# arogozhnikov/demuxalot

Hardware: AMD Instinct MI355X
Metric: EM iterations/sec + barcodes demuxed/sec, 200k bc x 100k SNP x 64 gt (higher is better)
Workload: dtype f32 terms, f64 sums (guarded mode: coarse pass reads the table as f16 and sums in f32; exact redo where the contract is not proven)

## Files before the change

### demuxalot_amd/_lib.py

```python
import ctypes
import os
from ctypes import POINTER, c_char_p, c_double, c_float, c_int, c_int32, c_int64, c_void_p

import numpy as np

_HERE = os.path.dirname(os.path.abspath(__file__))
LIB_PATH = os.environ.get('DEMUXALOT_AMD_LIB') or os.path.join(_HERE, 'libdemux_hip.so')

DMX_F32, DMX_F64 = 0, 1
T_PSTEP, T_ESTEP, T_MSTEP, T_MCOMBINE, T_ALLREDUCE, T_COUNT = 0, 1, 2, 3, 4, 5
TIMER_NAMES = ('pstep', 'estep', 'mstep', 'mcombine', 'allreduce')
HOST_COLLECTIVE = ctypes.CFUNCTYPE(ctypes.c_int, ctypes.c_void_p, ctypes.c_int, ctypes.c_void_p, ctypes.c_int64, ctypes.c_int)
COLL_ALL_REDUCE, COLL_REDUCE_SCATTER, COLL_ALL_GATHER = 0, 1, 2
UNIQUE_ID_BYTES = 128

_P = c_void_p
SIGNATURES = {
    'dmx_last_error': (c_char_p, []),
    'dmx_version': (c_char_p, []),
    'dmx_device_count': (c_int, [POINTER(c_int)]),
    'dmx_create': (c_int, [c_int, POINTER(_P)]),
    'dmx_destroy': (c_int, [_P]),
    'dmx_synchronize': (c_int, [_P]),
    'dmx_pack_calls_host': (c_int, [c_int64, _P, _P, _P, c_int64, _P, _P, _P, _P, _P, _P,
                                    POINTER(c_int64), POINTER(c_int64), _P, _P, _P, _P, _P]),
    'dmx_hash_host': (c_int, [_P, c_int64, c_int32, POINTER(ctypes.c_uint64)]),
    'dmx_set_problem': (c_int, [_P, c_int64, c_int64, c_int32, c_int64, _P, _P, _P, _P]),
    'dmx_pack_and_set_problem': (c_int, [_P, c_int64, c_int64, c_int32, _P, _P, _P, _P, c_int64, _P, _P, _P, _P, _P,
                                         POINTER(c_int64), POINTER(c_int64), _P]),
    'dmx_pack_containers_and_set_problem': (c_int, [_P, c_int64, c_int64, c_int32, _P, _P, _P, _P, _P, c_int32,
                                                    POINTER(c_int64), POINTER(c_int64), _P]),
    'dmx_stage_containers': (c_int, [_P, _P, c_int32]),
    'dmx_pack_staged_and_set_problem': (c_int, [_P, c_int64, c_int64, c_int32, _P, _P, _P, _P, _P, c_int32,
                                                POINTER(c_int64), POINTER(c_int64), _P]),
    'dmx_get_packed_calls': (c_int, [_P, _P, _P, _P, _P]),
    'dmx_set_betas': (c_int, [_P, _P]),
    'dmx_set_prior_betas': (c_int, [_P, _P, c_double, c_int, _P, _P]),
    'dmx_set_addition': (c_int, [_P, _P]),
    'dmx_probs_from_betas': (c_int, [_P, c_float, c_float, _P]),
    'dmx_probs_from_betas_f64': (c_int, [_P, _P, c_float, c_float, _P]),
    'dmx_set_probs': (c_int, [_P, _P]),
    'dmx_estep': (c_int, [_P, c_int, _P, _P, c_int, _P, _P]),
    'dmx_mstep': (c_int, [_P, c_float, _P]),
    'dmx_em': (c_int, [_P, c_int, c_float, c_float, c_int, _P, _P, c_int, c_float, _P, _P, _P]),
    'dmx_run_iterations': (c_int, [_P, c_int, c_float, c_float, c_float]),
    'dmx_get_logits': (c_int, [_P, _P]),
    'dmx_get_probs': (c_int, [_P, _P]),
    'dmx_get_addition': (c_int, [_P, _P]),
    'dmx_get_block': (c_int, [_P, c_int, c_int64, c_int64, c_int64, c_int64, _P]),
    'dmx_get_assignments': (c_int, [_P, _P, _P]),
    'dmx_get_assignments_above': (c_int, [_P, c_float, _P, _P, POINTER(c_int64)]),
    'dmx_get_top_options': (c_int, [_P, c_int32, _P, _P]),
    'dmx_get_option_sums': (c_int, [_P, _P]),
    'dmx_set_keep_molecule_calls': (c_int, [_P, c_int]),
    'dmx_set_molecule_calls': (c_int, [_P, c_int64, _P, _P, _P]),
    'dmx_get_max_pair_count': (c_int, [_P, POINTER(c_int64)]),
    'dmx_estep_snp': (c_int, [_P, c_int, _P, c_int64, _P, c_int, _P, _P]),
    'dmx_mstep_f64': (c_int, [_P, c_double, _P]),
    'dmx_mstep_f64_sums': (c_int, [_P, c_double, _P]),
    'dmx_get_prior_betas': (c_int, [_P, _P]),
    'dmx_get_learnt_betas': (c_int, [_P, _P]),
    'dmx_exchange_slices': (c_int, [c_int64, _P, c_int32, _P, POINTER(c_int64), POINTER(c_int32)]),
    'dmx_comm_unique_id': (c_int, [_P]),
    'dmx_comm_init': (c_int, [_P, c_int, c_int, _P, c_int]),
    'dmx_comm_init_host': (c_int, [_P, c_int, c_int, _P, _P, c_int]),
    'dmx_get_timings': (c_int, [_P, POINTER(c_double), POINTER(c_int64)]),
    'dmx_reset_timings': (c_int, [_P]),
    'dmx_set_phase_timers': (c_int, [_P, c_int]),
    'dmx_set_logits_needed': (c_int, [_P, c_int]),
    'dmx_set_lean_memory': (c_int, [_P, c_int]),
    'dmx_device_bytes': (c_int, [_P, POINTER(c_int64)]),
    'dmx_trim_cache': (c_int, [_P, POINTER(c_int64)]),
    'dmx_release_problem': (c_int, [_P]),
    'dmx_trim_device_caches': (c_int, [c_int, POINTER(c_int64)]),
    'dmx_set_exact_additions': (c_int, [_P, c_int]),
    'dmx_set_estep_mode': (c_int, [_P, c_int]),
    'dmx_set_msteps_expected': (c_int, [_P, c_int64]),
    'dmx_snp_count': (c_int, [_P, _P, c_int32, _P, c_int64, c_int32, c_float, c_int32, POINTER(c_int64)]),
    'dmx_snp_score': (c_int, [_P, c_double, _P, _P, _P, _P, _P, _P]),
    'dmx_snp_select': (c_int, [_P, c_int64, c_int64, _P, POINTER(c_int64)]),
    'dmx_count_reads': (c_int, [_P, _P, _P, c_int64, _P, POINTER(c_int64), POINTER(c_int64)]),
    'dmx_count_reads_fetch': (c_int, [_P, _P, _P]),
    'dmx_coverage_count': (c_int, [_P, _P, c_int32, c_int32, c_int32, _P]),
    'dmx_coverage_candidates': (c_int, [_P, c_double, c_double, c_double, c_double, c_int64, POINTER(c_int64)]),
    'dmx_coverage_fetch_candidates': (c_int, [_P, _P, _P]),
}
DEBUG_SIGNATURES = {
    'dmx_comm_init_emulated': (c_int, [_P, c_int, c_int, c_double, c_double, c_int]),
    'dmx_get_exchange_compact': (c_int, [_P, POINTER(c_int64), POINTER(c_int64), POINTER(c_int64)]),
    'dmx_get_exchange_compact_table': (c_int, [_P, POINTER(c_int64), POINTER(c_int64), POINTER(c_int64)]),
    'dmx_get_guard_probes': (c_int, [_P, POINTER(c_int64), POINTER(c_int64)]),
    'dmx_debug_set_pass_ms': (c_int, [_P, c_double, c_double, c_double]),
    'dmx_get_redo_count': (c_int, [_P, POINTER(c_int64)]),
    'dmx_set_guard_adaptive': (c_int, [_P, c_int]),
    'dmx_set_coarse_pass': (c_int, [_P, c_int]),
    'dmx_set_mstep_incremental': (c_int, [_P, c_int]),
    'dmx_get_mstep_incremental': (c_int, [_P, POINTER(c_int64), POINTER(c_int64), POINTER(c_int64)]),
    'dmx_get_guard_levels': (c_int, [_P, POINTER(c_int32), POINTER(c_int64), POINTER(c_int64), POINTER(c_int64), POINTER(c_double), POINTER(c_double), POINTER(c_double)]),
    'dmx_get_guard_direct': (c_int, [_P, POINTER(c_int32), POINTER(c_int64), POINTER(c_int64), POINTER(c_double), POINTER(c_double)]),
    'dmx_set_estep_schedule': (c_int, [_P, c_int]),
    'dmx_set_estep_dictionary': (c_int, [_P, c_int]),
    'dmx_get_estep_form': (c_int, [_P, POINTER(c_int32), POINTER(c_int32)]),
    'dmx_set_estep_packing': (c_int, [_P, c_int]),
    'dmx_set_mstep_wide_addresses': (c_int, [_P, c_int]),
    'dmx_set_mstep_tiles': (c_int, [_P, c_int]),
    'dmx_get_mstep_form': (c_int, [_P, POINTER(c_int32)]),
    'dmx_get_mstep_tiles_info': (c_int, [_P, POINTER(c_int32), POINTER(c_double)]),
    'dmx_test_logf': (c_int, [_P, _P, _P, c_int64]),
    'dmx_test_logf_hot': (c_int, [_P, _P, _P, c_int64]),
    'dmx_test_expf': (c_int, [_P, _P, _P, c_int64]),
    'dmx_test_log2_hw': (c_int, [_P, _P, _P, c_int64]),
    'dmx_test_softmax': (c_int, [_P, _P, _P, c_int64, c_int64]),
    'dmx_runtime_info': (c_int, [c_char_p, c_int64]),
    'dmx_get_exchange_mode': (c_int, [_P, POINTER(c_int32)]),
    'dmx_get_guard_stats': (c_int, [_P, POINTER(c_int64), POINTER(c_int64), POINTER(c_int64)]),
    'dmx_get_count_reads_timings': (c_int, [_P, POINTER(c_double)]),
    'dmx_count_reads_begin': (c_int, [_P, _P, c_int64, _P]),
    'dmx_count_reads_push': (c_int, [_P, _P, c_int, POINTER(c_int64), POINTER(c_int64)]),
    'dmx_count_reads_end': (c_int, [_P]),
    'dmx_get_count_reads_carry': (c_int, [_P, POINTER(c_int64)]),
    'dmx_get_count_reads_peak_bytes': (c_int, [_P, POINTER(c_int64)]),
    'dmx_set_coverage_form': (c_int, [_P, c_int]),
    'dmx_get_coverage_timings': (c_int, [_P, POINTER(c_double)]),
    'dmx_reads_upload': (c_int, [_P, _P, POINTER(c_int64)]),
    'dmx_reads_release': (c_int, [_P, c_int64]),
    'dmx_reads_info': (c_int, [_P, c_int64, POINTER(c_int64)]),
    'dmx_count_reads_resident': (c_int, [_P, c_int64, _P, c_int64, _P, POINTER(c_int64), POINTER(c_int64)]),
    'dmx_coverage_count_resident': (c_int, [_P, c_int64, c_int32, c_int32, c_int32, _P]),
    'dmx_count_reads_push_resident': (c_int, [_P, c_int64, c_int64, c_int64, c_int, POINTER(c_int64), POINTER(c_int64)]),
    'dmx_get_reads_upload_bytes': (c_int, [_P, POINTER(c_int64)]),
    'dmx_calls_upload': (c_int, [_P, _P, POINTER(c_int64)]),
    'dmx_calls_open': (c_int, [_P, POINTER(c_int64)]),
    'dmx_calls_append_counted': (c_int, [_P, c_int64]),
    'dmx_calls_seal': (c_int, [_P, c_int64]),
    'dmx_calls_concatenate': (c_int, [_P, POINTER(c_int64), c_int32, POINTER(c_int64)]),
    'dmx_calls_view': (c_int, [_P, c_int64, _P]),
    'dmx_calls_info': (c_int, [_P, c_int64, POINTER(c_int64)]),
    'dmx_calls_fetch': (c_int, [_P, c_int64, _P, _P]),
    'dmx_calls_release': (c_int, [_P, c_int64]),
    'dmx_calls_barcode_counts': (c_int, [_P, c_int64, c_int64, _P, _P]),
    'dmx_stage_device_containers': (c_int, [_P, _P, c_int32]),
    'dmx_snp_count_device': (c_int, [_P, _P, c_int32, _P, c_int64, c_int32, c_float, c_int32, POINTER(c_int64)]),
    'dmx_get_calls_transfer_bytes': (c_int, [_P, POINTER(c_int64)]),
    'dmx_get_donor_readout': (c_int, [_P, _P, _P, _P, _P, _P, _P, _P]),
    'dmx_get_allowed_mass': (c_int, [_P, _P, _P, _P, _P]),
    'dmx_estep_pools': (c_int, [_P, c_int, c_int32, _P, _P, _P, _P, _P, _P, _P, _P, _P, _P]),
    'dmx_estep_pools_resident': (c_int, [_P, c_int, c_int32, _P, _P, _P, _P, _P, _P, _P, _P, _P, _P]),
    'dmx_em_pools': (c_int, [_P, c_int, c_float, c_float, c_int, c_int32, _P, _P, _P, _P, _P, c_float, _P, _P, _P, _P, _P, _P]),
}

COVERAGE_STAGES = ('upload', 'walk', 'window', 'accumulate', 'filter', 'top_n')
COVERAGE_ATOMIC, COVERAGE_TILED = 0, 1
CALLS_INFO = ('n_molecules', 'n_snp_calls', 'nbytes', 'sealed')
READS_INFO = ('n_reads', 'n_cigar_ops', 'n_bases', 'nbytes', 'reference_length')
COUNT_READS_STAGES = ('upload', 'walk', 'molecules', 'duplicates', 'observations', 'fold', 'order')


class CallContainerStruct(ctypes.Structure):
    _fields_ = [('snp_calls', _P), ('n_snp_calls', c_int64), ('molecules', _P), ('n_molecules', c_int64), ('chrom', c_int32)]


class DecodedReadsStruct(ctypes.Structure):
    _fields_ = [('n_reads', c_int64), ('reference_start', _P), ('compressed_cb', _P), ('compressed_ub', _P), ('p_misaligned', _P),
                ('alignment_score', _P), ('cigar_begin', _P), ('n_cigar', _P), ('seq_begin', _P), ('l_seq', _P),
                ('n_cigar_ops', c_int64), ('cigar', _P), ('n_bases', c_int64), ('seq', _P), ('qual', _P)]


_lib = None


class DemuxHipError(RuntimeError):
    pass


def load():
    global _lib
    if _lib is None:
        if not os.path.exists(LIB_PATH):
            raise DemuxHipError(
                f'{LIB_PATH} is missing: build it with `python -c "import __graft_entry__ as g; g.build()"` '
                f'or `make -C demuxalot_amd/csrc`. demuxalot_amd has no CPU fallback.')
        os.environ.setdefault('HSA_ENABLE_IPC_MODE_LEGACY', '0')
        lib = ctypes.CDLL(LIB_PATH)
        for name, (res, args) in {**SIGNATURES, **DEBUG_SIGNATURES}.items():
            fn = getattr(lib, name)
            fn.restype = res
            fn.argtypes = args
        _lib = lib
    return _lib

# ... 35 lines not shown
```

### demuxalot_amd/csrc/dmx_api.cpp

```cpp
#include <dlfcn.h>
#include <hip/hip_runtime.h>
#include <rccl/rccl.h>

#include <array>
#include <chrono>
#include <functional>

#include <algorithm>
#include <mutex>
#include <cmath>
#include <cstdio>
#include <cstdlib>
#include <cstring>
#include <string>
#include <vector>

#include "dmx_ctx.h"
#include "dmx_host.h"

using namespace dmx::host;

extern "C" {

static int begin_problem(dmx_ctx *c, int64_t B, int64_t V, int32_t G, const int32_t *v2snp, std::vector<int> &snp_ptr,
// ... 345 lines not shown
        if (ms[i] < 0.0) continue;
        const unsigned ticks = (unsigned)std::min(ms[i] * (double)khz, 1.0e9);
        HIP_TRY(hipMemcpy(c->d_guard_count.p + word[i], &ticks, sizeof(unsigned), hipMemcpyHostToDevice));
        if (i == 2) {
            const unsigned measured = ticks != 0u;
            HIP_TRY(hipMemcpy(c->d_guard_count.p + dmx::GS_E_MEASURED, &measured, sizeof(unsigned), hipMemcpyHostToDevice));
        }
    }
    return 0;
}

int dmx_set_estep_dictionary(dmx_ctx *c, int mode)
{
    if (!c) return fail(DMX_ERR_INVALID, "null context");
    if (mode < 0 || mode > 2) return fail(DMX_ERR_INVALID, "dictionary mode must be 0, 1 or 2");
    c->dict_mode = mode;
    return 0;
}

int dmx_set_estep_packing(dmx_ctx *c, int on)
{
    if (!c) return fail(DMX_ERR_INVALID, "null context");
    if (on < 0 || on > 3) return fail(DMX_ERR_INVALID, "packing mode must be 0 .. 3");
    c->estep_packing = on;
    return 0;
}

int dmx_get_estep_form(dmx_ctx *c, int32_t *form, int32_t *distinct_values)
{
    if (!c) return fail(DMX_ERR_INVALID, "null context");
    if (form) *form = c->estep_form;
    if (distinct_values) *distinct_values = c->dict_distinct;
    return 0;
}

int dmx_set_estep_schedule(dmx_ctx *c, int tiled)
{
    if (!c) return fail(DMX_ERR_INVALID, "null context");
    if (tiled < 0 || tiled > 2) return fail(DMX_ERR_INVALID, "schedule must be 0, 1 or 2");
    c->tiled_estep = tiled;
    return 0;
}

int dmx_get_redo_count(dmx_ctx *c, int64_t *count)
{
    DMX_TRY(bind(c));
    if (!count) return fail(DMX_ERR_INVALID, "null argument");
    unsigned n[2] = {0, 0};
    if (c->d_n_redo.p) {
        HIP_TRY(hipMemcpyAsync(n, c->d_n_redo.p, 2 * sizeof(unsigned), hipMemcpyDeviceToHost, c->stream));
        HIP_TRY(hipStreamSynchronize(c->stream));
    }
    *count = (int64_t)n[0] + (int64_t)n[1];
    return 0;
}

int dmx_set_mstep_tiles(dmx_ctx *c, int enable)
{
    if (!c) return fail(DMX_ERR_INVALID, "null context");
    if (enable < 0 || enable > 2) return fail(DMX_ERR_INVALID, "dmx_set_mstep_tiles: 0 never, 1 when it pays, 2 always");
    c->mstep_tiles = enable;
    return 0;
}

int dmx_set_msteps_expected(dmx_ctx *c, int64_t n)
{
    if (!c) return fail(DMX_ERR_INVALID, "null context");
    c->msteps_expected = n > 0 ? (long long)n : 0;
    return 0;
}

int dmx_get_mstep_tiles_info(dmx_ctx *c, int32_t *built, double *build_ms)
{
    if (!c) return fail(DMX_ERR_INVALID, "null context");
    if (built) *built = c->n_mt > 0 ? 1 : 0;
    if (build_ms) *build_ms = c->n_mt > 0 ? c->mt_build_ms : 0.0;
    return 0;
}

int dmx_get_mstep_form(dmx_ctx *c, int32_t *form)
{
    if (!c || !form) return fail(DMX_ERR_INVALID, "null argument");
    *form = c->mstep_form;
    return 0;
}

int dmx_set_mstep_wide_addresses(dmx_ctx *c, int wide)
{
    if (!c) return fail(DMX_ERR_INVALID, "null context");
    c->mstep_wide = wide != 0;
    return 0;
}

int dmx_set_betas(dmx_ctx *c, const float *prior)
{
    DMX_TRY(bind(c));
    DMX_TRY(need(c, c->have_problem, "dmx_set_problem before dmx_set_betas"));
    if (!prior && c->V > 0) return fail(DMX_ERR_INVALID, "null betas");
    HIP_TRY(hipMemcpyAsync(c->d_prior.p, prior, sizeof(float) * c->V * c->G, hipMemcpyHostToDevice, c->stream));
    HIP_TRY(hipStreamSynchronize(c->stream));
    c->have_betas = true;
    c->have_raw = false;
    return 0;
}

int dmx_set_prior_betas(dmx_ctx *c, const float *raw_betas, double default_prior, int add_data_prior,
                        const int64_t *mol_per_variant, float *prior_out)
{
    DMX_TRY(bind(c));
    DMX_TRY(need(c, c->have_problem, "a resident problem before dmx_set_prior_betas"));
    const long long V = c->V;
    const int G = c->G;
    if (V > 0 && !raw_betas) return fail(DMX_ERR_INVALID, "null betas");
    const size_t vg = (size_t)V * G;
    c->have_raw = false;
    if (!c->d_raw.p) DMX_TRY(dev_alloc(c, c->d_raw, vg));
    float *d_raw = c->d_raw.p, *d_bsum = nullptr;
    HIP_TRY(hipMalloc((void **)&d_bsum, (size_t)(V ? V : 1) * sizeof(float)));
    int rc = 0;
    do {
        if (vg && hipMemcpyAsync(d_raw, raw_betas, vg * sizeof(float), hipMemcpyHostToDevice, c->stream) != hipSuccess) {
            rc = fail(DMX_ERR_HIP, "upload of the raw betas failed");
            break;
        }
        const unsigned long long *n_mol = nullptr;
        if (add_data_prior) {
            if (mol_per_variant) {
                dev_free(c, c->d_mol);
                if ((rc = dev_alloc(c, c->d_mol, (size_t)V)) != 0) break;
                if (V && hipMemcpyAsync(c->d_mol.p, mol_per_variant, sizeof(long long) * V, hipMemcpyHostToDevice, c->stream) != hipSuccess) {
                    rc = fail(DMX_ERR_HIP, "upload of the molecule counts failed");
                    break;
                }
            } else if (!c->d_mol.p) {
                rc = fail(DMX_ERR_INVALID, "add_data_prior needs molecule counts: pass them or install the problem with dmx_pack_and_set_problem");
                break;
            }
            n_mol = c->d_mol.p;
        }
        const hipError_t e = dmx::launch_prior_betas(c->stream, d_raw, d_bsum, n_mol, c->d_v2snp.p, c->d_snp_ptr.p, c->d_snp_vars.p, V, G,
                                    default_prior, c->d_prior.p);
        if (e != hipSuccess) {
            rc = fail(DMX_ERR_HIP, "prior betas kernel: %s", hipGetErrorString(e));
            break;
        }
        if (prior_out && vg && hipMemcpyAsync(prior_out, c->d_prior.p, vg * sizeof(float), hipMemcpyDeviceToHost, c->stream) != hipSuccess) {
            rc = fail(DMX_ERR_HIP, "download of the prior betas failed");
            break;
        }
        if (hipStreamSynchronize(c->stream) != hipSuccess) rc = fail(DMX_ERR_HIP, "synchronisation failed");
    } while (false);
    (void)hipStreamSynchronize(c->stream);
    (void)hipFree(d_bsum);
    if (rc == 0) c->have_betas = c->have_raw = true;
    return rc;
}

int dmx_get_prior_betas(dmx_ctx *c, float *out)
{
    DMX_TRY(bind(c));
    DMX_TRY(need(c, c->have_problem && c->have_betas, "prior betas (dmx_set_betas / dmx_set_prior_betas) before dmx_get_prior_betas"));
    DMX_TRY(copy_out(c, out, c->d_prior.p, (size_t)c->V * c->G));
    HIP_TRY(hipStreamSynchronize(c->stream));
    return 0;
}

// ... 123 lines not shown
```

### demuxalot_amd/csrc/dmx_ctx.h

```cpp
#pragma once
#include <hip/hip_runtime.h>
#include <rccl/rccl.h>

#include <map>
#include <mutex>
#include <string>
#include <unordered_map>
#include <utility>
#include <vector>

#include "dmx_internal.h"
#include "kernels.h"

using dmx::fail;

#define HIP_TRY(expr)                                                                                   \
    do {                                                                                                \
        hipError_t _e = (expr);                                                                         \
        if (_e != hipSuccess) return fail(DMX_ERR_HIP, "%s failed: %s", #expr, hipGetErrorString(_e)); \
    } while (0)

#define DMX_TRY(expr)         \
    do {                      \
        int _s = (expr);      \
// ... 98 lines not shown
    DevBuf<unsigned> d_coarse_stream;
    DevBuf<long long> d_coarse_bin_ptr;
    DevBuf<double> d_log2_keep;
    bool coarse_ready = false;
    bool prob16_valid = false;
    int coarse_pass = 1;
    int lean_memory = 0;
    bool logits_needed = true;
    bool logits_readable = true;
    float p_clip_lo = 0.0f;
    DevBuf<double> d_add64, d_partial;
    DevBuf<float> d_logits, d_post;
    DevBuf<unsigned long long> d_nz;
    DevBuf<unsigned long long> d_redo;
    DevBuf<unsigned> d_n_redo;
    bool mstep_wide = false;
    DevBuf<uint2> d_mt_stream;
    DevBuf<long long> d_mt_ptr;
    DevBuf<int> d_mt_first;
    DevBuf<int> d_mt_order;
    DevBuf<int> d_mt_shift;
    DevBuf<unsigned char> d_mt_shift_v;
    DevBuf<unsigned long long> d_acc64;
    DevBuf<float> d_prev_post;
    DevBuf<uint2> d_prev_first;
    DevBuf<int> d_incr_list;
    DevBuf<unsigned char> d_incr_touched;
    DevBuf<unsigned> d_incr_state;
    int incr_parity = 0;
    bool incr_valid = false;
    float incr_power = 0.0f;
    int mstep_incremental = 1;
    long long mstep_incr_launches = 0;
    long long n_mt = 0;
    std::vector<long long> h_col_ptr;
    int mt_tv = 0;
    bool mt_tried = false;
    bool mt_shift_tried = false;
    int mstep_tiles = 1;
    long long msteps_done = 0;
    long long incr_rows = 0;
    DevBuf<unsigned char> d_incr_map;
    DevBuf<uint2> d_slice_rec;
    DevBuf<long long> d_slice_ptr;
    bool slice_index_tried = false;
    bool incr_heavy = false;
    int msteps_ahead = 0;
    long long msteps_expected = 0;
    double mt_build_ms = 0.0;
    int mstep_form = 0;
    DevBuf<int> d_sum_plan;
    long long sum_plan_k = -1;
    int sum_plan_values = 0;
    int item_calls = 1024;
    bool exact_additions = true;
    int estep_mode = DMX_ESTEP_EXACT;
    DevBuf<unsigned> d_guard_count;
    int guard_adaptive = 1;
    DevBuf<int> d_guard_list;
    DevBuf<int> d_guard_sub;
    unsigned guard_sub_cap = 0;
    long long guard_rows_total = 0;
    bool guard_ran = false;
    int tiled_estep = 1;
    int dict_mode = 1;
    bool add_is_zero = true;
    bool dict_candidate = false;
    int estep_form = 0;
    int estep_packing = 1;
    long long max_row_calls = 0;
    int n_simd = 0;
    long long long_row_calls[3] = {0, 0, 0};
    long long n_long_rows[3] = {0, 0, 0};
    int dict_distinct = 0;
    DevBuf<float> d_dict;
    DevBuf<unsigned char> d_codes;
    DevBuf<unsigned char> d_dtab;
    DevBuf<unsigned> d_dict_stat;
    DevBuf<dmx::EstepSegment> d_segs;
    DevBuf<int> d_split_first;
    DevBuf<double> d_seg_sums;
    long long n_segs = 0, n_split = 0;
    float nz_floor = 0.0f;
    DevBuf<uint2> d_first;
    DevBuf<unsigned long long> d_dense_calls;
    bool dense_stat_valid = false;
    DevBuf<float> d_pen;
    DevBuf<unsigned> d_pairs;
    DevBuf<unsigned> d_pair_blocks;
    int n_pair_blocks = 0;
    DevBuf<unsigned char> d_prior_logits;
    DevBuf<int> d_best;
    DevBuf<float> d_bestp;
    DevBuf<int> d_u_variant, d_u_cb;
    DevBuf<float> d_u_p;
    DevBuf<long long> d_u_count;
    long long n_u = 0;
    DevBuf<unsigned long long> d_mol;
    bool keep_molecule_calls = false;
    DevBuf<int> d_mc_variant;
    DevBuf<float> d_mc_e;
    DevBuf<long long> d_mc_start;
    unsigned mc_max_count = 0;
    DevBuf<double> d_logits64, d_post64;
    bool have_post64 = false;
    DevBuf<unsigned char> d_scratch;
    DevBuf<unsigned long long> d_sd_pos;
    DevBuf<int> d_sd_counts;
    DevBuf<double> d_sd_imp;
    long long sd_P = -1;
    int sd_D = 0;
    bool sd_scored = false;
    DevBuf<unsigned char> d_cr_molecules;
    DevBuf<unsigned char> d_cr_calls;
    long long cr_molecules = -1, cr_calls = 0;
    double cr_stage_ms[dmx::COUNT_READS_STAGES] = {};
    int64_t cr_peak_bytes = 0;
    long long cr_carried = 0;
    DevBuf<int> d_crs_positions;
    DevBuf<double> d_crs_table;
    ReadColumns crs_carry;
    int crs_state = 0;
    long long crs_P = 0;
    long long crs_molecules = 0;
    long long crs_previous_start = 0;
    bool crs_has_previous = false;
    DevBuf<int> d_cov_counts;
    DevBuf<int> d_cov_cand_pos;
    DevBuf<int> d_cov_cand_counts;
    long long cov_W = -1, cov_start = 0, cov_candidates = -1;
    int coverage_form = DMX_COVERAGE_TILED;
    double cov_stage_ms[dmx::COVERAGE_STAGES] = {};
    std::map<int64_t, ResidentReads> resident_reads;
    int64_t reads_upload_bytes = 0;
    std::map<int64_t, ResidentCalls> resident_calls;
    int64_t calls_transfer_bytes[2] = {0, 0};

    ncclComm_t comm = nullptr;
    dmx_host_collective host_coll = nullptr;
    void *host_user = nullptr;
    void *h_stage = nullptr;
    size_t h_stage_bytes = 0;
    bool emulated = false;
    double emu_link_gbps = 50.0, emu_latency_us = 10.0;
    bool in_group = false, group_paid = false;
    double group_ns = 0.0;
    bool emu_table_filled = false;
    double emu_ticks_per_ns = 0.1;
    bool attached() const { return comm != nullptr || host_coll != nullptr || emulated; }
    int rank = 0, nranks = 1, reduce_dtype = DMX_F64;
    bool sliced = false;
    bool add_partial = false;
    long long slice_rows = 0;
    long long prob_rows = 0;
    std::vector<long long> cut;
    std::vector<int> h_v2snp;
    DevBuf<int> d_prow;
    DevBuf<int> d_row_variant;
    bool mshard = false;
    long long rows_pad = 0, rows_total = 0;
    DevBuf<uint2> d_first_g;
    DevBuf<unsigned long long> d_nz_g;
    DevBuf<float> d_post_g;
    bool post_gathered = false;
    bool emu_post_filled = false;
    DevBuf<unsigned> d_post_compact;
// ... 129 lines not shown
```

### demuxalot_amd/csrc/dmx_runtime.cpp

```cpp
#include <dlfcn.h>
#include <hip/hip_runtime.h>
#include <rccl/rccl.h>

#include <array>
#include <chrono>
#include <functional>

#include <algorithm>
#include <mutex>
#include <cmath>
#include <cstdio>
#include <cstdlib>
#include <cstring>
#include <string>
#include <vector>

#include "dmx_ctx.h"
#include "dmx_host.h"

using namespace dmx::host;

namespace dmx {
static thread_local std::string g_last_error;

// ... 677 lines not shown
    c->boundary = nullptr;
    for (int slot = 0; slot < DMX_T_COUNT; slot++) timer_flush(c, slot);
    for (TimerStamp *s : c->idle_stamps) {
        (void)hipEventDestroy(s->ev);
        delete s;
    }
    (void)hipStreamDestroy(c->stream);
    delete c;
    return 0;
}

int dmx_synchronize(dmx_ctx *c)
{
    DMX_TRY(bind(c));
    HIP_TRY(hipStreamSynchronize(c->stream));
    return 0;
}

int dmx_release_problem(dmx_ctx *c)
{
    DMX_TRY(bind(c));
    HIP_TRY(hipStreamSynchronize(c->stream));
    release_problem(c);
    release_snp_detection(c);
    release_count_reads(c);
    release_count_reads_stream(c);
    release_coverage(c);
    dmx::release_staged_calls(c);
    return 0;
}

int dmx_trim_device_caches(int device, int64_t *released_bytes)
{
    int n = 0;
    if (hipGetDeviceCount(&n) != hipSuccess || device < 0 || device >= n) return fail(DMX_ERR_INVALID, "device %d out of range", device);
    HIP_TRY(hipSetDevice(device));
    const size_t freed = trim_device_caches(device);
    if (released_bytes) *released_bytes = (int64_t)freed;
    return 0;
}

int dmx_trim_cache(dmx_ctx *c, int64_t *released_bytes)
{
    DMX_TRY(bind(c));
    size_t before = 0;
    {
        std::lock_guard<std::mutex> own(c->cache_lock);
        before = c->idle_bytes;
    }
    ctx_trim(c, 0);
    before += retired_trim(c->device);
    if (released_bytes) *released_bytes = (int64_t)before;
    return 0;
}

int dmx_set_phase_timers(dmx_ctx *c, int on)
{
    if (!c) return fail(DMX_ERR_INVALID, "null ctx");
    c->phase_timers = on != 0;
    c->boundary = nullptr;
    return 0;
}

int dmx_get_timings(dmx_ctx *c, double *ms, int64_t *launches)
{
    DMX_TRY(bind(c));
    HIP_TRY(hipStreamSynchronize(c->stream));
    for (int s = 0; s < DMX_T_COUNT; s++) {
        timer_flush(c, s);
        if (ms) ms[s] = (c->timers[s].launches > 0 && c->timers[s].timed == 0) ? -1.0 : c->timers[s].ms;
        if (launches) launches[s] = c->timers[s].launches;
    }
    return 0;
}

int dmx_reset_timings(dmx_ctx *c)
{
    DMX_TRY(bind(c));
    HIP_TRY(hipStreamSynchronize(c->stream));
    if (c->d_guard_count.p) HIP_TRY(hipMemsetAsync(c->d_guard_count.p + dmx::GS_PENDING, 0, 4 * sizeof(unsigned), c->stream));
    if (c->d_guard_count.p) HIP_TRY(hipMemsetAsync(c->d_guard_count.p + dmx::GS_COARSE_STEPS, 0, 2 * sizeof(unsigned), c->stream));
    if (c->d_incr_state.p) HIP_TRY(hipMemsetAsync(c->d_incr_state.p + 2 * dmx::IS_WORDS, 0, sizeof(unsigned) * 3, c->stream));
    c->guard_rows_total = 0;
    for (int s = 0; s < DMX_T_COUNT; s++) {
        timer_flush(c, s);
        c->timers[s].ms = 0.0;
        c->timers[s].launches = 0;
        c->timers[s].timed = 0;
    }
    return 0;
}

int dmx_device_bytes(dmx_ctx *c, int64_t *bytes)
{
    if (!c || !bytes) return fail(DMX_ERR_INVALID, "null argument");
    *bytes = c->bytes;
    return 0;
}

}
```

### demuxalot_amd/csrc/dmx_steps.cpp

```cpp
#include <dlfcn.h>
#include <hip/hip_runtime.h>
#include <rccl/rccl.h>

#include <array>
#include <chrono>
#include <functional>

#include <algorithm>
#include <mutex>
#include <cmath>
#include <cstdio>
#include <cstdlib>
#include <cstring>
#include <string>
#include <vector>

#include "dmx_ctx.h"
#include "dmx_host.h"
#include "estep_plan.h"
#include "estep_pools.h"
#include "mstep_plan.h"

using namespace dmx::host;

// ... 213 lines not shown
    c->dict_candidate = !with_addition || c->add_is_zero;
    return 0;
}

namespace ep = dmx::eplan;
static_assert(ep::MODE_EXACT == DMX_ESTEP_EXACT && ep::MODE_FAST == DMX_ESTEP_FAST && ep::MODE_GUARDED == DMX_ESTEP_GUARDED, "estep_plan.h: Mode");

static ep::Facts estep_facts(const dmx_ctx *c, int with_doublets, bool with_prior, bool logits_kept)
{
    ep::Facts f{};
    f.mode = (ep::Mode)c->estep_mode;
    f.with_doublets = with_doublets != 0;
    f.with_prior = with_prior;
    f.logits_kept = logits_kept;
    f.G = c->G;
    f.K = c->K;
    f.B = c->B;
    f.table_rows = c->prob_rows;
    f.schedule = c->tiled_estep;
    f.n_bins = c->n_bins;
    f.tile_stream = c->d_tile_stream.p != nullptr;
    f.coarse_ready = c->coarse_ready;
    f.coarse_pass = c->coarse_pass;
    f.guard_adaptive = c->guard_adaptive != 0;
    f.lean_memory = c->lean_memory != 0;
    f.lo = c->p_clip_lo;
    f.prob16_valid = c->prob16_valid;
    f.sliced = c->sliced;
    f.table_lists = c->prob_list_words != 0;
    f.dict_mode = c->dict_mode;
    f.dict_candidate = c->dict_candidate;
    f.call_rows = c->d_call_rows.p != nullptr;
    f.records_below_4g = ((unsigned long long)c->n_pairs + dmx::CALL_PAD_PAIRS) * sizeof(dmx::CallPair) < (1ull << 32);
    f.packing = c->estep_packing;
    f.row_statistic = c->max_row_calls > 0;
    for (int k = 0; k < 3; k++) f.n_long_rows[k] = c->n_long_rows[k];
    f.segments = c->n_segs > 0;
    f.n_pair_blocks = with_doublets && c->d_pair_blocks.p != nullptr ? c->n_pair_blocks : 0;
    return f;
}

int prepare_dictionary(dmx_ctx *c, bool pairs, dmx::EstepArgs &a, int *form)
{
    const ep::Facts f = estep_facts(c, pairs, false, true);
    *form = DMX_FORM_DIRECT;
    a.dict_n = 0;
    c->dict_distinct = 0;
    if (!ep::dictionary_admissible(f)) return 0;
    const int G = c->G;
    const long long K = c->K, rows = c->prob_rows;
    const size_t code_pitch = (size_t)dmx::dict_code_pitch(G);
    DMX_TRY(dev_grow(c, c->d_dict, (size_t)rows * dmx::DICT_CAP));
    DMX_TRY(dev_grow(c, c->d_codes, (size_t)rows * code_pitch));
    if (!c->d_dict_stat.p) DMX_TRY(dev_alloc(c, c->d_dict_stat, (size_t)1));
    HIP_TRY(dmx::launch_build_dict(c->stream, c->d_prob.p, rows, G, c->d_dict.p, c->d_codes.p, c->d_dict_stat.p));
    unsigned distinct = 0;
    HIP_TRY(hipMemcpyAsync(&distinct, c->d_dict_stat.p, sizeof(unsigned), hipMemcpyDeviceToHost, c->stream));
    HIP_TRY(hipStreamSynchronize(c->stream));
    c->dict_distinct = (int)distinct;
    const size_t pitch = ep::dictionary_candidate_form(f, distinct) == ep::DICT_LANE ? (size_t)dmx::dict_table_pitch((int)distinct, (int)K, f.with_doublets) : 0;
    switch (ep::dictionary_form(f, distinct, pitch)) {
    case ep::DICT_NONE:
        return 0;
    case ep::DICT_BLOCK:
        a.dict_n = (int)distinct;
        a.dict = c->d_dict.p;
        a.codes = c->d_codes.p;
        *form = DMX_FORM_DICT_BLOCK;
        return 0;
    case ep::DICT_LANE:
        break;
    }
    const size_t need_bytes = (size_t)rows * pitch;
    DMX_TRY(dev_grow(c, c->d_dtab, need_bytes));
    HIP_TRY(dmx::launch_pack_rows(c->stream, c->d_dict.p, c->d_codes.p, c->d_pairs.p, rows, G, (int)K, f.with_doublets, (int)distinct, c->d_dtab.p));
    a.dict_n = (int)distinct;
    a.dtab = c->d_dtab.p;
    a.dtab_pitch = (int)pitch;
    a.dtab_bytes = (unsigned)need_bytes;
    *form = DMX_FORM_DICT;
    return 0;
}

static void fill_estep_args(dmx_ctx *c, dmx::EstepArgs &a, int with_doublets, bool with_prior, int prior_dtype, float power)
{
    a.pair_ptr = c->d_pair_ptr.p;
    a.order = c->d_bc_order.p;
    a.pairs = c->d_call_pairs.p;
    a.call_rows = c->d_call_rows.p;
    const unsigned long long rec_bytes = ((unsigned long long)c->n_pairs + dmx::CALL_PAD_PAIRS) * sizeof(dmx::CallPair);
    a.pairs_bytes = rec_bytes < (1ull << 32) ? (unsigned)rec_bytes : 0u;
    a.prob = c->d_prob.p;
    a.prob16 = nullptr;
    a.guard_accum = 0.0f;
    a.guard_alt_per_call = 0.0f;
    a.guard_alt_accum = 0.0f;
    a.guard_main_coarse = 0;
    a.opt_pairs = c->d_pairs.p;
    a.pair_blocks = with_doublets ? c->d_pair_blocks.p : nullptr;
    a.n_pair_blocks = with_doublets ? c->n_pair_blocks : 0;
    a.sum_plan = c->d_sum_plan.p;
    a.sum_plan_values = c->sum_plan_values;
    a.pen = c->d_pen.p;
    a.prior = with_prior ? c->d_prior_logits.p : nullptr;
    a.prior_dtype = prior_dtype;
    a.logits = c->d_logits.p;
    a.post = c->d_post.p;
    const size_t row_base = c->mshard ? (size_t)c->rank * (size_t)c->rows_pad : 0;
    a.nz = c->mshard ? c->d_nz_g.p + row_base * ((c->G + 63) / 64) : c->d_nz.p;
    a.first = c->G <= 64 ? (c->mshard ? c->d_first_g.p + row_base : c->d_first.p) : nullptr;
    a.post_singlets = c->mshard ? c->d_post_g.p + row_base * c->G : nullptr;
    a.dense_calls = c->G <= 64 ? c->d_dense_calls.p : nullptr;
    a.nz_floor = power == 2.0f ? dmx::NZ_FLOOR_SQUARE : 0.0f;
    a.B = c->B;
    a.prob_bytes = (unsigned)((unsigned long long)c->prob_rows * c->G * 4ull);
    a.G = c->G;
    a.K = c->K;
    a.fast = 0;
    a.guard = 0;
    a.guard_per_call = ep::GUARD_PER_CALL_PLAIN;
    a.guard_count = c->d_guard_count.p;
    a.guard_list = c->d_guard_list.p;
    a.guard_sub = c->d_guard_sub.p;
    a.guard_sub_cap = c->guard_sub_cap;
    a.order_count = nullptr;
    a.direct = nullptr;
    a.order_direct = nullptr;
    a.segs = nullptr;
    a.n_segs = c->n_segs;
    a.n_split = c->n_split;
    a.split_first = c->d_split_first.p;
    a.seg_sums = c->d_seg_sums.p;
    a.tiled = c->tiled_estep;
    a.n_bins = 0;
    a.bin_rows_cap = c->bin_rows_cap;
    a.bin_order = c->d_bin_order.p;
    a.bin_rows = c->d_bin_rows.p;
    a.bin_ptr = c->d_bin_ptr.p;
    a.tile_stream = c->d_tile_stream.p;
    a.coarse_stream = nullptr;
    a.coarse_bin_ptr = nullptr;
    a.log2_keep = nullptr;
    a.n_long = 0;
    a.dict_n = 0;
    a.dtab = nullptr;
    a.dtab_bytes = 0;
    a.dtab_pitch = 0;
    a.dict = nullptr;
    a.codes = nullptr;
}

static void set_walk(const dmx_ctx *c, dmx::EstepArgs &a, ep::Walk walk, bool coarse = false)
{
    const ep::Handover h = ep::handover(walk, coarse);
    a.tile_stream = c->d_tile_stream.p;
    if (!h.bins) a.n_bins = 0;
    if (h.coarse_records) {
        a.coarse_stream = c->d_coarse_stream.p;
        a.coarse_bin_ptr = c->d_coarse_bin_ptr.p;
        a.log2_keep = c->d_log2_keep.p;
    }
    if (h.prob16) a.prob16 = c->d_prob16.p;
}

static int guarded_estep(dmx_ctx *c, ep::Facts &f, dmx::EstepArgs &a)
{
    const bool capable = ep::coarse_capable(f, f.lo), allow_coarse = ep::allow_coarse(f), release = ep::lean_release_due(f);
    const float fine_allowance_found = ep::fine_allowance(f, ep::walk(f));
    if (ep::coarse_build_due(f)) {
        const int cpg = ep::coarse_calls_per_gather(f.K), bpr = ep::coarse_batches_per_record(cpg);
        const size_t words = (((size_t)c->n_pairs / 4 + (size_t)c->n_bins * (bpr - 1)) / bpr + 1) * (size_t)(cpg * 16);
        DMX_TRY(dev_alloc(c, c->d_coarse_stream, words));
        DMX_TRY(dev_alloc(c, c->d_coarse_bin_ptr, (size_t)c->n_bins + 1));
        DMX_TRY(dev_alloc(c, c->d_log2_keep, (size_t)c->B));
        HIP_TRY(dmx::launch_build_coarse_stream(c->stream, c->d_tile_stream.p, c->d_bin_ptr.p, c->n_bins, a.prob_bytes, cpg, c->d_coarse_bin_ptr.p, c->d_coarse_stream.p,
                                                c->d_bin_rows.p, c->bin_rows_cap, c->d_log2_keep.p));
        c->coarse_ready = f.coarse_ready = true;
        if (release) {
            dev_free(c, c->d_tile_stream);
            dev_free(c, c->d_call_rows);
            a.tile_stream = nullptr;
            a.call_rows = nullptr;
            f.tile_stream = f.call_rows = false;
        }
    }
    if (allow_coarse) DMX_TRY(ensure_prob16(c));
    HIP_TRY(dmx::launch_guard_begin(c->stream, c->d_guard_count.p, c->B, c->K, c->guard_adaptive, capable, allow_coarse));
    a.guard = 1;
    a.guard_per_call = fine_allowance_found;
    a.order_direct = c->d_bc_order.p;
    a.guard_main_coarse = 0;
    a.guard_alt_per_call = capable ? dmx::GUARD_PER_CALL_COARSE : 0.0f;
    a.guard_alt_accum = capable ? dmx::GUARD_ACCUM_F32 : 0.0f;
    if (allow_coarse) {
        if (ep::prob16_conversion_due(f)) {
            const bool kept = ep::prob16_stays_valid(f);
// ... 68 lines not shown
            HIP_TRY(dmx::launch_estep_packed(c->stream, a));
            form = DMX_FORM_PACKED;
        } else if (ep::guarded(f)) {
            DMX_TRY(guarded_estep(c, f, a));
        } else {
            set_walk(c, a, ep::walk(f));
            HIP_TRY(dmx::launch_estep(c->stream, a, f.with_doublets));
        }
    }
    c->estep_form = form;
    if (a.dense_calls) HIP_TRY(dmx::launch_sum_dense(c->stream, c->d_dense_calls.p, c->guard_ran ? c->d_guard_count.p : nullptr));
    else if (c->guard_ran) HIP_TRY(dmx::launch_guard_stamp(c->stream, c->d_guard_count.p, dmx::GS_T_END));
    timer_end(c, DMX_T_ESTEP, ev);
    c->have_post = true;
    c->logits_readable = logits_kept;
    return 0;
}

static int ensure_incremental_state(dmx_ctx *c, bool sharded, long long incr_rows, float power)
{
    if (!c->d_acc64.p) {
        c->incr_rows = incr_rows;
        DMX_TRY(dev_alloc(c, c->d_acc64, (size_t)c->V * c->G));
        DMX_TRY(dev_alloc(c, c->d_prev_post, (size_t)incr_rows * c->G));
        DMX_TRY(dev_alloc(c, c->d_prev_first, (size_t)incr_rows));
        DMX_TRY(dev_alloc(c, c->d_incr_list, (size_t)incr_rows));
        if (sharded) {
            DMX_TRY(dmx::build_slice_row_index(c));
            if (c->d_slice_rec.p == nullptr) {
                DMX_TRY(dev_alloc(c, c->d_incr_map, (size_t)incr_rows));
                HIP_TRY(hipMemsetAsync(c->d_incr_map.p, 0, (size_t)incr_rows, c->stream));
            }
        }
        DMX_TRY(dev_alloc(c, c->d_incr_touched, (size_t)c->V));
        DMX_TRY(dev_alloc(c, c->d_incr_state, (size_t)(3 * dmx::IS_WORDS)));
        HIP_TRY(hipMemsetAsync(c->d_incr_state.p, 0, sizeof(unsigned) * 3 * dmx::IS_WORDS, c->stream));
        HIP_TRY(hipMemsetAsync(c->d_incr_touched.p, 0, (size_t)c->V, c->stream));
        c->incr_valid = false;
    }
    if (!c->incr_valid || c->incr_power != power) {
        HIP_TRY(hipMemsetAsync(c->d_incr_state.p, 0, sizeof(unsigned) * 2 * dmx::IS_WORDS, c->stream));
        if (c->mstep_incremental == 2 && !c->attached()) {
            const unsigned on[2] = {1u, 1u};
            HIP_TRY(hipMemsetAsync(c->d_acc64.p, 0, sizeof(unsigned long long) * (size_t)c->V * c->G, c->stream));
            HIP_TRY(hipMemsetAsync(c->d_prev_post.p, 0, sizeof(float) * (size_t)incr_rows * c->G, c->stream));
            HIP_TRY(hipMemsetAsync(c->d_prev_first.p, 0xFF, sizeof(uint2) * (size_t)incr_rows, c->stream));
            HIP_TRY(hipMemsetAsync(c->d_add.p, 0, sizeof(float) * (size_t)c->V * c->G, c->stream));
            HIP_TRY(hipMemcpyAsync(c->d_incr_state.p + dmx::IS_VALID, &on[0], sizeof(unsigned), hipMemcpyHostToDevice, c->stream));
            HIP_TRY(hipMemcpyAsync(c->d_incr_state.p + dmx::IS_FORCE, &on[1], sizeof(unsigned), hipMemcpyHostToDevice, c->stream));
            HIP_TRY(hipStreamSynchronize(c->stream));
        }
        c->incr_parity = 0;
        c->incr_valid = true;
        c->incr_power = power;
    }
    return 0;
}

int run_mstep(dmx_ctx *c, float power)
{
    const bool mshard = c->mshard;
    const size_t row_base = mshard ? (size_t)c->rank * (size_t)c->rows_pad : 0;
    const int Wn = (c->G + 63) / 64;
    dmx::MstepArgs a;
    a.order = c->d_item_order.p;
    a.item_start = c->d_item_start.p;
    a.item_len = c->d_item_len.p;
    a.calls = c->d_csc.p;
    a.post = mshard ? c->d_post_g.p : c->d_post.p;
    a.nz = mshard ? c->d_nz_g.p : c->d_nz.p;
    a.first = mshard ? c->d_first_g.p : c->d_first.p;
    const unsigned long long rows = mshard ? (unsigned long long)c->rows_total : (unsigned long long)c->B;
    a.K = mshard ? c->G : c->K;
    a.first_bytes = 8ull * rows;
    a.wide = c->mstep_wide;
    a.post_bytes = rows * (unsigned long long)a.K * 4ull;
    a.partial = c->d_partial.p;
    a.n_items = c->n_items;
    a.G = c->G;
    a.square = (power == 2.0f);
    a.power = power;
    a.dense_calls = c->dense_stat_valid && a.post_bytes < (1ull << 32) ? c->d_dense_calls.p : nullptr;
    a.total_calls = 2ull * (unsigned long long)c->n_pairs;
    if (!a.square && c->nz_floor != 0.0f) {
        HIP_TRY(dmx::launch_rebuild_nz(c->stream, c->d_post.p, c->B, c->K, c->G, 0.0f, (mshard ? c->d_nz_g.p : c->d_nz.p) + row_base * Wn,
                                       c->G <= 64 ? (mshard ? c->d_first_g.p : c->d_first.p) + row_base : nullptr));
        c->nz_floor = 0.0f;
        c->post_gathered = false;
    }
    DMX_TRY(gather_posteriors(c));
    c->add_is_zero = false;
    TimerSpan ev{nullptr, nullptr};
    SpanGuard ev_guard{c, &ev};
    mplan::Facts f{};
    f.mstep_tiles = c->mstep_tiles;
    f.mstep_incremental = c->mstep_incremental;
    f.exact_additions = c->exact_additions;
    f.G = c->G;
    f.has_calls = c->n_csc > 0;
    f.power = power;
    f.attached = c->attached();
    f.mshard = c->mshard;
    f.sliced = c->sliced;
    f.reduce_f64 = c->reduce_dtype == DMX_F64;
    f.has_call_pairs = c->d_call_pairs.p != nullptr;
    f.has_item_variant = c->d_item_variant.p != nullptr;
    f.has_shift_v = c->d_mt_shift_v.p != nullptr;
    f.has_incr_state = c->d_incr_state.p != nullptr;
    f.has_slice_rec = c->d_slice_rec.p != nullptr;
    f.n_mt = c->n_mt;
    f.mt_tried = c->mt_tried;
    f.msteps_done = c->msteps_done;
    f.msteps_ahead = c->msteps_ahead;
    f.msteps_expected = c->msteps_expected;
    f.incr_heavy = c->incr_heavy;
    f.rows_total = c->rows_total;
    if (mplan::probe_due(f)) {
        unsigned full_passes = 0;
        HIP_TRY(hipMemcpyAsync(&full_passes, c->d_incr_state.p + 2 * dmx::IS_WORDS + 3, sizeof(unsigned), hipMemcpyDeviceToHost, c->stream));
        HIP_TRY(hipStreamSynchronize(c->stream));
        f.incr_heavy = c->incr_heavy = mplan::heavy_after_probe(f, full_passes);
    }
    if (c->msteps_expected > 0) c->msteps_expected--;
    c->msteps_done++;
    const mplan::Range own = mplan::variant_range(f, c->cut.data(), c->rank, c->V);
    if (mplan::build_due(f)) {
        HIP_TRY(hipStreamSynchronize(c->stream));
        const auto t0 = std::chrono::steady_clock::now();
        DMX_TRY(dmx::build_mstep_tiles(c, own.v0, own.v1));
        c->mt_build_ms = std::chrono::duration<double, std::milli>(std::chrono::steady_clock::now() - t0).count();
        f.n_mt = c->n_mt;
    }
    if (mplan::shifts_wanted(f)) DMX_TRY(dmx::plan_mstep_shifts(c));
    f.has_shift_v = c->d_mt_shift_v.p != nullptr;
    const mplan::Launch plan = mplan::launch(f);
    const mplan::Dest dest = mplan::destination(f);
    const bool incremental = plan.incr != mplan::INCR_NONE, sharded = plan.incr == mplan::INCR_SHARDED;
    const long long incr_rows = sharded ? c->rows_total : c->B;
    if (incremental) DMX_TRY(ensure_incremental_state(c, sharded, incr_rows, power));
    else c->incr_valid = false;
    f.has_slice_rec = c->d_slice_rec.p != nullptr;
    const bool by_rows = sharded && mplan::sharded_by_row_index(f);
    a.item_variant = c->d_item_variant.p;
    a.item_ptr = c->d_item_ptr.p;
    a.prow = dest.exchange_buffer ? c->d_prow.p : nullptr;
    a.out32 = dest.f64 ? nullptr : dest.exchange_buffer ? (float *)c->d_exch.p : c->d_add.p;
    a.out64 = !dest.f64 ? nullptr : dest.exchange_buffer ? (double *)c->d_exch.p : c->d_add64.p;
    a.redo_cap = c->d_redo.n;
    a.tiles_done = plan.form == 2;
    a.incr_total = !sharded ? 0ull : by_rows ? (unsigned long long)c->n_csc : 2ull * (unsigned long long)incr_rows;
    dmx::MTileArgs tiles{};
    if (a.tiles_done) {
        tiles.stream = c->d_mt_stream.p;
        tiles.ptr = c->d_mt_ptr.p;
        tiles.first = c->d_mt_first.p;
        tiles.order = c->d_mt_order.p;
        tiles.shift = c->d_mt_shift.p;
        tiles.n_tiles = c->n_mt;
        tiles.tv = c->mt_tv;
    }
    dmx::MIncrArgs incr{};
    if (incremental) {
        incr.state = c->d_incr_state.p + c->incr_parity * dmx::IS_WORDS;
        incr.next = c->d_incr_state.p + (c->incr_parity ^ 1) * dmx::IS_WORDS;
        c->incr_parity ^= 1;
        incr.counters = c->d_incr_state.p + 2 * dmx::IS_WORDS;
        incr.acc64 = c->d_acc64.p;
        incr.prev = c->d_prev_post.p;
        incr.prev_first = c->d_prev_first.p;
        incr.list = c->d_incr_list.p;
        incr.touched = c->d_incr_touched.p;
        incr.shift_v = c->d_mt_shift_v.p;
        incr.pairs = sharded ? nullptr : c->d_call_pairs.p;
        incr.call_rows = sharded ? nullptr : c->d_call_rows.p;
        incr.pair_ptr = sharded ? nullptr : c->d_pair_ptr.p;
        incr.changed_map = sharded ? c->d_incr_map.p : nullptr;
        incr.rec = sharded ? c->d_slice_rec.p : nullptr;
        incr.rec_ptr = by_rows ? c->d_slice_ptr.p : nullptr;
        incr.row_variant = plan.row_variant ? c->d_row_variant.p : nullptr;
        incr.B = incr_rows;
        incr.V = c->V;
        incr.floor = dmx::mincr_floor(power);
        tiles.acc64 = c->d_acc64.p;
        tiles.incr_state = incr.state;
        c->mstep_incr_launches++;
    }
    const bool fixed = plan.incr == mplan::INCR_WORK_ITEMS;
    a.fixed_shift_v = fixed ? c->d_mt_shift_v.p : nullptr;
    a.fixed_acc64 = fixed ? c->d_acc64.p : nullptr;
    a.fixed_state = fixed ? incr.state : nullptr;
    timer_begin(c, DMX_T_MSTEP, &ev);
    HIP_TRY(incremental ? dmx::launch_mstep_incremental(c->stream, a, a.tiles_done ? &tiles : nullptr, incr)
            : a.tiles_done ? dmx::launch_mstep_tiles(c->stream, a, tiles) : dmx::launch_mstep(c->stream, a));
    c->mstep_form = plan.form;
    timer_end(c, DMX_T_MSTEP, ev);
    timer_begin(c, DMX_T_MCOMBINE, &ev);
    HIP_TRY(dmx::launch_mcombine(c->stream, a, c->d_item_ptr.p, own.v0, own.v1, a.prow, a.out32, a.out64, c->exact_additions ? c->d_redo.p : nullptr,
                                 c->d_n_redo.p, nullptr, true));
    timer_end(c, DMX_T_MCOMBINE, ev);
    int rc = 0;
    if (dest.then != mplan::EXCH_NONE) timer_begin(c, DMX_T_ALLREDUCE, &ev);
    if (dest.then == mplan::EXCH_REDUCE_SCATTER) {
        rc = coll_reduce_scatter(c, c->d_exch.p, c->d_recv.p, (size_t)c->slice_rows * c->G, dest.f64, c->stream);
        if (rc == 0)
            HIP_TRY(dmx::launch_store_slice(c->stream, c->d_recv.p, dest.f64, c->cut[c->rank], c->cut[c->rank + 1] - c->cut[c->rank], c->G, c->d_add.p));
    } else if (dest.then == mplan::EXCH_ALL_REDUCE) {
        rc = coll_all_reduce(c, dest.f64 ? (void *)c->d_add64.p : (void *)c->d_add.p, (size_t)c->V * c->G, dest.f64);
        if (rc == 0 && dest.f64) HIP_TRY(dmx::launch_f64_to_f32(c->stream, c->d_add64.p, c->d_add.p, (long long)c->V * c->G));
    }
    if (dest.then != mplan::EXCH_NONE) timer_end(c, DMX_T_ALLREDUCE, ev);
    if (rc == 0 && dest.slice_only) c->add_partial = c->nranks > 1;
    return rc;
}

}
}

extern "C" {

// ... 136 lines not shown
        if (p < -1 || p >= n_pools) return fail(DMX_ERR_INVALID, "%s: pool_of_barcode[%lld] = %d is outside [-1, %d)", who, b, p, (int)n_pools);
        const long long options = p < 0 ? 0 : plan.opt_ptr[(size_t)p + 1] - plan.opt_ptr[(size_t)p];
        if (row_ptr[b + 1] - row_ptr[b] != options)
            return fail(DMX_ERR_INVALID, "%s: row_ptr gives barcode %lld %lld entries, its pool has %lld options", who, b,
                        (long long)(row_ptr[b + 1] - row_ptr[b]), options);
    }
    plan.pair_penalty = pair_penalty;
    plan.pool_of_barcode = pool_of_barcode;
    plan.row_ptr = row_ptr;
    plan.logits_out = logits_out;
    plan.probs_out = probs_out;
    plan.best_option = best_option;
    plan.best_prob = best_prob;
    plan.doublet_mass = doublet_mass;
    return 0;
}

static int begin_dense_pools(dmx_ctx *c)
{
    const std::vector<float> zeros((size_t)std::max(c->G, 1), 0.0f);
    DMX_TRY(ensure_options(c, 0, zeros.data()));
    const size_t bg = (size_t)c->B * c->G;
    HIP_TRY(hipMemsetAsync(c->d_post.p, 0, sizeof(float) * (bg ? bg : 1), c->stream));
    c->have_post = false;
    return 0;
}

int dmx_estep_pools(dmx_ctx *c, int with_doublets, int32_t n_pools, const int64_t *pool_start, const int32_t *pool_donors,
                    const float *pair_penalty, const int32_t *pool_of_barcode, const int64_t *row_ptr, float *logits_out,
                    float *probs_out, int32_t *best_option, float *best_prob, double *doublet_mass)
{
    DMX_TRY(bind(c));
    dmx::PoolsPlan plan;
    DMX_TRY(plan_pools(c, "dmx_estep_pools", false, false, with_doublets, n_pools, pool_start, pool_donors, pair_penalty, pool_of_barcode, row_ptr,
                       logits_out, probs_out, best_option, best_prob, doublet_mass, plan));
    return dmx::run_estep_pools(c, plan);
}

int dmx_estep_pools_resident(dmx_ctx *c, int with_doublets, int32_t n_pools, const int64_t *pool_start, const int32_t *pool_donors,
                             const float *pair_penalty, const int32_t *pool_of_barcode, const int64_t *row_ptr, float *logits_out,
                             float *probs_out, int32_t *best_option, float *best_prob, double *doublet_mass)
{
    DMX_TRY(bind(c));
    dmx::PoolsPlan plan;
    DMX_TRY(plan_pools(c, "dmx_estep_pools_resident", true, false, with_doublets, n_pools, pool_start, pool_donors, pair_penalty, pool_of_barcode,
                       row_ptr, logits_out, probs_out, best_option, best_prob, doublet_mass, plan));
    DMX_TRY(begin_dense_pools(c));
    dmx::PoolsRunPtr run;
    DMX_TRY(dmx::prepare_estep_pools(c, plan, true, run));
    DMX_TRY(dmx::launch_estep_pools_pass(c, *run, 2.0f));
    return dmx::read_back_estep_pools(c, *run);
}

int dmx_mstep(dmx_ctx *c, float power, float *addition_out)
{
    DMX_TRY(bind(c));
    DMX_TRY(need(c, c->have_problem && c->have_post, "dmx_estep before dmx_mstep"));
    DMX_TRY(run_mstep(c, power));
    if (addition_out) DMX_TRY(ensure_full_addition(c));
    DMX_TRY(copy_out(c, addition_out, c->d_add.p, (size_t)c->V * c->G));
    HIP_TRY(hipStreamSynchronize(c->stream));
    return 0;
}

int dmx_em(dmx_ctx *c, int n_iterations, float lo, float hi, int with_doublets, const float *penalties,
           const void *prior_logits, int prior_dtype, float power, float *logits_out, float *probs_out,
           float *addition_out)
{
    DMX_TRY(bind(c));
    DMX_TRY(need(c, c->have_problem && c->have_betas, "dmx_set_problem + dmx_set_betas before dmx_em"));
    if (n_iterations < 1) return fail(DMX_ERR_INVALID, "n_iterations must be >= 1");
    if (!penalties) return fail(DMX_ERR_INVALID, "null penalties");
    DMX_TRY(ensure_options(c, with_doublets, penalties));
    DMX_TRY(upload_prior_logits(c, prior_logits, prior_dtype));
    const size_t vg = (size_t)c->V * c->G;
    HIP_TRY(hipMemsetAsync(c->d_add.p, 0, sizeof(float) * (vg ? vg : 1), c->stream));
    c->incr_valid = false;
    c->add_is_zero = true;
    c->add_partial = false;
    const bool keep_last = c->logits_needed || logits_out != nullptr;
    for (int it = 0; it < n_iterations; it++) {
        const bool kept = it + 1 == n_iterations && keep_last;
        DMX_TRY(run_pstep(c, lo, hi, true, !kept && it > 0 && ep::coarse_capable(estep_facts(c, with_doublets, false, kept), lo)));
        DMX_TRY(run_estep(c, with_doublets, it == 0 && prior_logits != nullptr, prior_dtype, power, kept));
        if (it + 1 < n_iterations) {
            c->msteps_ahead = n_iterations - 1 - it;
            const int rc_m = run_mstep(c, power);
            c->msteps_ahead = 0;
            if (rc_m) return rc_m;
        }
    }
    const size_t bk = (size_t)c->B * c->K;
    DMX_TRY(copy_out(c, logits_out, c->d_logits.p, bk));
    DMX_TRY(copy_out(c, probs_out, c->d_post.p, bk));
    DMX_TRY(ensure_full_addition(c));
    DMX_TRY(copy_out(c, addition_out, c->d_add.p, vg));
    HIP_TRY(hipStreamSynchronize(c->stream));
    return 0;
}

int dmx_em_pools(dmx_ctx *c, int n_iterations, float lo, float hi, int with_doublets, int32_t n_pools, const int64_t *pool_start,
                 const int32_t *pool_donors, const float *pair_penalty, const int32_t *pool_of_barcode, const int64_t *row_ptr, float power,
                 float *logits_out, float *probs_out, int32_t *best_option, float *best_prob, double *doublet_mass, float *addition_out)
{
    DMX_TRY(bind(c));
    dmx::PoolsPlan plan;
    DMX_TRY(plan_pools(c, "dmx_em_pools", true, true, with_doublets, n_pools, pool_start, pool_donors, pair_penalty, pool_of_barcode, row_ptr,
                       logits_out, probs_out, best_option, best_prob, doublet_mass, plan));
    if (n_iterations < 1) return fail(DMX_ERR_INVALID, "dmx_em_pools: n_iterations must be >= 1");
    DMX_TRY(begin_dense_pools(c));
    const size_t vg = (size_t)c->V * c->G;
    HIP_TRY(hipMemsetAsync(c->d_add.p, 0, sizeof(float) * (vg ? vg : 1), c->stream));
    c->incr_valid = false;
    c->add_is_zero = true;
    c->add_partial = false;
    dmx::PoolsRunPtr run;
    DMX_TRY(dmx::prepare_estep_pools(c, plan, true, run));
    for (int it = 0; it < n_iterations; it++) {
        DMX_TRY(run_pstep(c, lo, hi, true, false));
        DMX_TRY(dmx::launch_estep_pools_pass(c, *run, power));
        if (it + 1 < n_iterations) {
            c->msteps_ahead = n_iterations - 1 - it;
            const int rc_m = run_mstep(c, power);
            c->msteps_ahead = 0;
            if (rc_m) return rc_m;
        }
    }
    DMX_TRY(copy_out(c, addition_out, c->d_add.p, vg));
    return dmx::read_back_estep_pools(c, *run);
}

int dmx_run_iterations(dmx_ctx *c, int n_iterations, float lo, float hi, float power)
{
    DMX_TRY(bind(c));
    DMX_TRY(need(c, c->have_problem && c->have_betas && c->have_post && c->K > 0,
                 "dmx_estep or dmx_em (to fix the options) before dmx_run_iterations"));
    if (n_iterations < 0) return fail(DMX_ERR_INVALID, "negative n_iterations");
    const int with_doublets = c->K != c->G;
    for (int it = 0; it < n_iterations; it++) {
        const bool kept = it + 1 == n_iterations && c->logits_needed;
        DMX_TRY(run_pstep(c, lo, hi, true, !kept && ep::coarse_capable(estep_facts(c, with_doublets, false, kept), lo)));
        DMX_TRY(run_estep(c, with_doublets, false, DMX_F32, power, kept));
        c->msteps_ahead = n_iterations - it;
        const int rc_m = run_mstep(c, power);
        c->msteps_ahead = 0;
        if (rc_m) return rc_m;
    }
    return 0;
}

}
```

### demuxalot_amd/csrc/estep_epilogue.h

```cpp
#pragma once
#include <hip/hip_runtime.h>

#include "kernels.h"
#include "np_math.h"

namespace dmx {

static __device__ __forceinline__ double shfl_xor_f64(double v, int mask)
{
    int lo = __double2loint(v), hi = __double2hiint(v);
    lo = __shfl_xor(lo, mask);
    hi = __shfl_xor(hi, mask);
    return __hiloint2double(hi, lo);
}

constexpr int NZ_CODE = 4;
__device__ __forceinline__ uint2 nz_code(unsigned long long live, float first_posterior)
{
    unsigned code = (unsigned)__popcll(live);
#pragma unroll
    for (int t = 0; t < NZ_CODE; t++) {
        if (live) code |= (unsigned)__builtin_ctzll(live) << (7 + 6 * t);
        live &= live - 1ull;
    }
// ... 154 lines not shown
constexpr float GUARD_PER_CALL = 7.0e-8f;
constexpr float GUARD_PER_CALL_PRESCALED = 3.1e-7f;
constexpr float GUARD_LOGIT_ROUNDING = 1.2e-7f;
constexpr int GUARD_ALT_SAMPLE = 8;
constexpr float GUARD_TOL = 8.0e-6f;
constexpr float GUARD_TOL_WIDE = 6.0e-6f;

template <int L, int A>
static __device__ __forceinline__ bool estep_guard(const float (&dev)[A], const float (&lg)[A], const float (&post)[A],
                                                   const bool (&valid)[A], float mx, int gbase)
{
    float dmax = 0.0f;
    bool bad = false;
#pragma unroll
    for (int s = 0; s < A; s++) {
        if (!valid[s]) continue;
        bad |= !(dev[s] < 40.0f);
        dmax = fmaxf(dmax, dev[s]);
    }
#pragma unroll
    for (int off = 1; off < L; off <<= 1) dmax = fmaxf(dmax, __shfl_xor(dmax, off));
    const float x2 = 2.0f * dmax;
    const float e2 = dmax < 0.25f ? x2 * (1.0f + x2) * 1.000001f : __builtin_amdgcn_exp2f(x2 * 1.4426953f) * 1.00002f - 1.0f;
    const float near = mx - (x2 + 2.4e-7f * fabsf(mx)) * 1.000001f;
    int close = 0;
#pragma unroll
    for (int s = 0; s < A; s++) {
        const float m = fminf(post[s], 1.0f - post[s]);
        bad |= valid[s] && !(m * e2 <= GUARD_TOL);
        const unsigned long long bal = __ballot(valid[s] && !(lg[s] < near));
        close += __popcll(L == 64 ? bal : (bal >> gbase) & group_mask<L>());
    }
    const unsigned long long any_bad = __ballot(bad);
    return close != 1 || (L == 64 ? any_bad : (any_bad >> gbase) & group_mask<L>()) != 0ull;
}

static __device__ __forceinline__ void guard_note(const EstepArgs &a, long long b, bool counting, bool coarse_set = false)
{
    if (counting) {
        atomicAdd(a.guard_count + (coarse_set ? GS_SLOTS_COARSE : GS_SLOTS_FINE) + (int)(b & (GUARD_SLOTS - 1)), 1u);
    } else {
        const unsigned q = (unsigned)(b & (GUARD_QUEUES - 1));
        a.guard_sub[(size_t)q * a.guard_sub_cap + atomicAdd(a.guard_count + GS_QUEUE_LEN + q, 1u)] = (int)b;
    }
}
static __device__ __forceinline__ bool guard_stand_back(const EstepArgs &a)
{
    return a.guard == 1 && a.direct != nullptr && *a.direct != 0u;
}
static __device__ __forceinline__ bool guard_active(const EstepArgs &a)
{
    return a.guard == 1 || (a.guard == 2 && a.direct != nullptr && *a.direct != 0u);
}

template <int L, int A, bool GUARD = false>
static __device__ __forceinline__ void estep_epilogue(const EstepArgs &a, long long b, bool live, const double (&acc)[A],
                                                      const int (&kk)[A], const bool (&valid)[A], int lane, int li, int gbase,
                                                      int row_calls, float accum_extra = 0.0f)
{
    const int K = a.K;
    float lg[A], x[A];
    float mx = -__builtin_inff();
#pragma unroll
    for (int s = 0; s < A; s++) {
        const double t = (double)a.pen[kk[s]] + acc[s];
        float l = (float)t;
        if (a.prior) {
            const size_t o = (size_t)b * K + kk[s];
            if (a.prior_dtype == DMX_F32)
                l = l + ((const float *)a.prior)[o];
            else
                l = (float)((double)l + ((const double *)a.prior)[o]);
        }
        lg[s] = l;
        mx = valid[s] ? fmaxf(mx, l) : mx;
    }
#pragma unroll
    for (int off = 1; off < L; off <<= 1) mx = fmaxf(mx, __shfl_xor(mx, off));
#pragma unroll
    for (int s = 0; s < A; s++) x[s] = npm::exp_f32(lg[s] - mx);
    const float tot = reg_row_sum<L, A>(x, K, lane, gbase);
    const int W = (a.G + 63) >> 6;
    unsigned long long mine = 0ull;
    float post[A];
#pragma unroll
    for (int s = 0; s < A; s++) {
        post[s] = x[s] / tot;
        if (live && valid[s]) {
            const size_t o = (size_t)b * K + kk[s];
            a.logits[o] = lg[s];
            a.post[o] = post[s];
            if (a.post_singlets != nullptr && kk[s] < a.G) a.post_singlets[(size_t)b * a.G + kk[s]] = post[s];
        }
        const unsigned long long bal = __ballot(live && valid[s] && (li + L * s) < a.G && !(post[s] <= a.nz_floor));
        if (L == 64) {
            if (lane == 0 && s < W) a.nz[(size_t)b * W + s] = bal;
            if (s == 0) mine = bal;
        } else if (L * s < 64) {
            mine |= ((bal >> gbase) & group_mask<L>()) << ((L * s) & 63);
        }
    }
    if (L < 64 && live && li == 0) a.nz[(size_t)b] = mine;
    bool redo = false;
    if (a.guard && guard_active(a)) {
        const bool counting = a.guard == 2;
        float dev[A];
        const float n = (float)row_calls;
        auto bound = [&](float per_call, float accum) {
#pragma unroll
            for (int s = 0; s < A; s++) {
                const float l0 = (float)((double)a.pen[kk[s]] + acc[s]);
                dev[s] = GUARD_RHO * (fabsf((float)acc[s]) + GUARD_POSITIVE_TERM * n) + per_call * (n + 8.0f) + GUARD_LOGIT_ROUNDING * fabsf(l0);
                if (accum != 0.0f) dev[s] += accum * (0.125f * n + 2.0f) * (fabsf((float)acc[s]) + 3.0e-4f * n + accum_extra);
                if (a.prior) dev[s] += GUARD_LOGIT_ROUNDING * fabsf(lg[s]);
            }
        };
        bound(a.guard_per_call, a.guard_accum);
        const bool flagged = estep_guard<L, A>(dev, lg, post, valid, mx, gbase);
        if (flagged && live && li == 0) guard_note(a, b, counting, a.guard_main_coarse != 0);
        redo = flagged && !counting;
        if (a.guard_alt_per_call != 0.0f && (L < 64 || (b & (GUARD_ALT_SAMPLE - 1)) == 0)) {
            bound(a.guard_alt_per_call, a.guard_alt_accum);
            const bool flagged_alt = estep_guard<L, A>(dev, lg, post, valid, mx, gbase);
            if (flagged_alt && live && li == 0 && (b & (GUARD_ALT_SAMPLE - 1)) == 0)
                atomicAdd(a.guard_count + (a.guard_main_coarse == 0 ? GS_SLOTS_COARSE : GS_SLOTS_FINE) + (int)((b / GUARD_ALT_SAMPLE) & (GUARD_SLOTS - 1)), (unsigned)GUARD_ALT_SAMPLE);
        }
    }
    if (a.first) {
        const int g0 = mine ? __builtin_ctzll(mine) : 0;
        float p0 = post[0];
#pragma unroll
        for (int s = 1; s < A; s++) p0 = (g0 >> log2_lanes<L>()) == s ? post[s] : p0;
        if (live && li == (g0 & (L - 1))) a.first[b] = nz_code(mine, p0);
        if (a.dense_calls && live && !redo && li == 0 && __popcll(mine) > 4)
            atomicAdd(a.dense_calls + 1 + (b & (DENSE_SLOTS - 1)), (unsigned long long)row_calls);
    }
}

}
```

### demuxalot_amd/csrc/kernels.h

```cpp
#pragma once
#include <hip/hip_runtime.h>

#include "demux_hip.h"
#include "demux_hip_debug.h"
#include "estep_plan.h"

namespace dmx {

struct alignas(32) CallPair {
    unsigned row_off[2];
    float keep[2];
    float floor[2];
    unsigned reserved[2];
};
static_assert(sizeof(CallPair) == 32, "CallPair layout");

#ifndef DMX_PAIRBLOCK_R1
#define DMX_PAIRBLOCK_R1 2
#define DMX_PAIRBLOCK_R2 3
#endif
constexpr int PAIRBLOCK_R1 = DMX_PAIRBLOCK_R1, PAIRBLOCK_R2 = DMX_PAIRBLOCK_R2;

struct EstepSegment {
    int barcode;
    int first_pair;
    int n_pairs;
    int pad;
};

struct EstepArgs {
    const long long *pair_ptr;
    const int *order;
    const CallPair *pairs;
    const unsigned *call_rows;
    unsigned pairs_bytes;
    const float *prob;
    const unsigned short *prob16;
    const int *sum_plan;
    int sum_plan_values;
    const unsigned *opt_pairs;
    const unsigned *pair_blocks;
    int n_pair_blocks;
    const float *pen;
    const void *prior;
    int prior_dtype;
    float *logits;
    float *post;
    float *post_singlets;
    unsigned long long *nz;
    uint2 *first;
    float nz_floor;
    unsigned long long *dense_calls;
    long long B;
    unsigned prob_bytes;
    int G;
    int K;
    int fast;
    float guard_accum;
    float guard_alt_per_call;
    float guard_alt_accum;
    int guard_main_coarse;
    float guard_per_call;
    int guard;
    unsigned *guard_count;
    int *guard_list;
    int *guard_sub;
    unsigned guard_sub_cap;
    const unsigned *order_count;
    const unsigned *direct;
    const int *order_direct;
    const EstepSegment *segs;
    long long n_segs;
    long long n_split;
    const int *split_first;
    double *seg_sums;
    int tiled;
    long long n_bins;
    int bin_rows_cap;
    const int *bin_order;
    const int *bin_rows;
    const long long *bin_ptr;
    const unsigned *coarse_stream;
    const long long *coarse_bin_ptr;
    const double *log2_keep;
    const CallPair *tile_stream;
    int dict_n;
    const unsigned char *dtab;
    unsigned dtab_bytes;
    int dtab_pitch;
    long long n_long;
    const float *dict;
    const unsigned char *codes;
};

enum { GS_COUNT = 0,
       GS_DIRECT = 1,
       GS_VALID = 2,
       GS_ROWS = 3,
       GS_PENDING = 4,
       GS_DIRECT_STEPS = 5,
       GS_TOTAL = 6,
       GS_T_FAST = 8,
       GS_T_REDO = 9,
       GS_T_END = 10,
       GS_F_TICKS = 11,
       GS_E_TICKS = 12,
       GS_E_MEASURED = 13,
       GS_O_TICKS = 14,
       GS_K = 15,
       GS_LEVEL = 16,
       GS_SKIP_COARSE = 17,
       GS_SKIP_FINE = 18,
       GS_C_TICKS = 19,
       GS_COUNT_FINE = 20,
       GS_COUNT_COARSE = 21,
       GS_CAPABLE = 22,
       GS_COARSE_STEPS = 23,
       GS_PROBES = 24,
       GS_STREAK = 25,
       GS_WORDS = 26 };
constexpr unsigned GUARD_PROBE_STREAK = 64;
constexpr unsigned GS_UNKNOWN = 0xFFFFFFFFu;
constexpr float GUARD_PER_CALL_COARSE = 5.1e-4f;
using eplan::guard_per_call_fine8;
constexpr float GUARD_ACCUM_F32 = 6.0e-8f;
constexpr int GUARD_SLOTS = 256;
constexpr int GUARD_QUEUES = 256;
constexpr int GS_SLOTS_FINE = GS_WORDS, GS_SLOTS_COARSE = GS_WORDS + GUARD_SLOTS, GS_QUEUE_LEN = GS_WORDS + 2 * GUARD_SLOTS;
constexpr int GUARD_STATE_WORDS = GS_WORDS + 2 * GUARD_SLOTS + GUARD_QUEUES;
hipError_t launch_guard_compact(hipStream_t st, unsigned *state, const int *sub, unsigned sub_cap, int *list, const int *order_direct, long long B);
hipError_t launch_guard_begin(hipStream_t st, unsigned *state, long long B, int K, int adaptive, int capable, int allow_coarse);
hipError_t launch_guard_stamp(hipStream_t st, unsigned *state, int which);

constexpr int CALL_PAD_PAIRS = 64;
using eplan::DICT_CAP;
using eplan::DICT_PAIR_CAP;
using eplan::DICT_LANE_K;
__host__ __device__ inline int dict_code_pitch(int n) { return (n + 3) & ~3; }

constexpr int DENSE_SLOTS = 1024;
hipError_t launch_sum_dense(hipStream_t st, unsigned long long *counters, unsigned *guard_state = nullptr);
constexpr int TILE_R_MAX = 9;
constexpr long long TILE_BYTES = 1 << 20;
#ifndef DMX_TILE_MIN_BARCODES
#define DMX_TILE_MIN_BARCODES 8192
#endif
constexpr long long TILE_MIN_BARCODES = DMX_TILE_MIN_BARCODES;
#ifndef DMX_TILE_MIN_TABLE_BYTES
#define DMX_TILE_MIN_TABLE_BYTES (1 << 20)
#endif
constexpr long long TILE_MIN_TABLE_BYTES = DMX_TILE_MIN_TABLE_BYTES;

struct MstepArgs {
    const int *order;
    const long long *item_start;
    const int *item_len;
    const uint2 *calls;
    const float *post;
    const unsigned long long *nz;
    bool wide;
    unsigned long long first_bytes;
    const uint2 *first;
    double *partial;
    const int *item_variant;
    unsigned long long redo_cap;
    bool tiles_done;
    const long long *item_ptr;
    const int *prow;
    float *out32;
    double *out64;
    long long n_items;
    long long K;
    unsigned long long post_bytes;
    int G;
    int square;
    float power;
    const unsigned long long *dense_calls;
    unsigned long long total_calls;
    const unsigned char *fixed_shift_v;
    unsigned long long *fixed_acc64;
    const unsigned *fixed_state;
    unsigned long long incr_total;
};

constexpr float NZ_FLOOR_SQUARE = 8.271806125530277e-25f;

constexpr int MIN_ITEM_CALLS = 1024, MAX_ITEM_CALLS = 16384;
inline int item_calls_for(long long n_calls)
{
    long long len = MIN_ITEM_CALLS;
    while (len < MAX_ITEM_CALLS && len * 6000 < n_calls) len *= 2;
    return (int)len;
}

hipError_t launch_probs_from_betas(hipStream_t st, const float *prior, const float *addition, const int *v2snp,
                                   const int *snp_ptr, const int *snp_vars, long long v_begin, long long n_rows, long long n_snps,
                                   int G, const int *prow, float lo, float hi, float *prob, unsigned short *prob16 = nullptr);
hipError_t launch_probs_from_betas_f64(hipStream_t st, const double *betas, const int *v2snp, const int *snp_ptr,
                                       const int *snp_vars, long long V, long long n_snps, int G, const int *prow, float lo,
                                       float hi, float *prob);
hipError_t launch_check_unit_range(hipStream_t st, const float *x, long long n, int *flags);
hipError_t launch_estep(hipStream_t st, const EstepArgs &a, bool pairs);
using eplan::coarse_calls_per_gather;
using eplan::coarse_batches_per_record;
hipError_t launch_build_coarse_stream(hipStream_t st, const CallPair *stream, const long long *bin_ptr, long long n_bins, unsigned zero_off,
                                      int cpg, long long *coarse_bin_ptr, unsigned *out, const int *bin_rows, int R, double *log2_keep);
hipError_t launch_prob_to_half(hipStream_t st, const float *prob, long long rows, int G, unsigned short *out, const unsigned *skip);
hipError_t launch_softmax_rows(hipStream_t st, const EstepArgs &a);
hipError_t launch_build_dict(hipStream_t st, const float *prob, long long rows, int G, float *dict, unsigned char *codes, unsigned *stat);
int dict_table_pitch(int distinct, int K, bool pairs);
hipError_t launch_pack_rows(hipStream_t st, const float *dict, const unsigned char *codes, const unsigned *opt_pairs, long long rows, int G,
                            int K, bool pairs, int distinct, unsigned char *table);
hipError_t launch_estep_dict(hipStream_t st, const EstepArgs &a, bool pairs);
hipError_t launch_estep_dict_block(hipStream_t st, const EstepArgs &a);
hipError_t launch_mstep(hipStream_t st, const MstepArgs &a);
struct MTileArgs {
    const uint2 *stream;
    const long long *ptr;
    const int *first;
    const int *order;
    const int *shift;
    long long n_tiles;
    int tv;
    unsigned long long *acc64;
    const unsigned *incr_state;
};
struct MIncrArgs {
    unsigned *state;
    unsigned *next;
    unsigned *counters;
    unsigned long long *acc64;
    float *prev;
    uint2 *prev_first;
    int *list;
    unsigned char *touched;
    const unsigned char *shift_v;
    const CallPair *pairs;
    const unsigned *call_rows;
    const long long *pair_ptr;
    long long B, V;
    float floor;
    unsigned char *changed_map;
    const int *row_variant;
    const uint2 *rec;
    const long long *rec_ptr;
};
enum { IS_N = 0,
       IS_CALLS = 2,
       IS_VALID = 4,
       IS_STREAK = 5,
       IS_SITOUT = 6,
       IS_FORCE = 7,
       IS_WORDS = 8 };
inline float mincr_floor(float power) { return power * 126.0f > 52.0f ? exp2f(-52.0f / power) : 0.0f; }
hipError_t launch_mstep_incremental(hipStream_t st, const MstepArgs &a, const MTileArgs *t, const MIncrArgs &x);
constexpr int MTILE_LDS_BYTES = 64 * 1024;
constexpr int MTILE_MAX_VARIANTS = 128;
hipError_t launch_mstep_tiles(hipStream_t st, const MstepArgs &a, const MTileArgs &t);

hipError_t launch_mcombine(hipStream_t st, const MstepArgs &a, const long long *item_ptr, long long v0, long long v1,
                           const int *prow, float *add32, double *add64, unsigned long long *redo, unsigned *n_redo,
                           const int *vlist = nullptr, bool skip_single = false);
hipError_t launch_store_slice(hipStream_t st, const void *slice, bool f64, long long v_begin, long long n_rows, int G, float *add);
using eplan::estep_packed_shape;
hipError_t launch_estep_packed(hipStream_t st, const EstepArgs &a);
hipError_t launch_remap_row_offsets(hipStream_t st, CallPair *pairs, long long n_pairs, unsigned row_bytes, const int *new_rows,
                                    unsigned *call_rows);
hipError_t launch_f64_to_f32(hipStream_t st, const double *in, float *out, long long n);
hipError_t launch_add_f32(hipStream_t st, const float *a, const float *b, float *out, long long n);
hipError_t launch_delay(hipStream_t st, long long ticks);
hipError_t launch_post_compact_build(hipStream_t st, const uint2 *first, const float *post, long long B, int G, unsigned cap, unsigned *block,
                                     float *sent, unsigned char *sent_multi, unsigned *peers, unsigned long long block_words, int nranks, int own);
hipError_t launch_prob_changes_build(hipStream_t st, const float *slice, float *prev, long long rows, int G, unsigned cap, unsigned *block,
                                     unsigned *peers, unsigned long long block_words, int nranks, int own);
hipError_t launch_prob_changes_apply(hipStream_t st, float *table, const unsigned *blocks, unsigned long long block_words, long long slice_rows, int G,
                                     int nranks, int own, unsigned cap, unsigned short *table16);
hipError_t launch_post_counts(hipStream_t st, const unsigned *blocks, unsigned long long block_words, int nranks, unsigned *out_host_visible, unsigned seq);
hipError_t launch_post_reconstruct(hipStream_t st, const uint2 *first_g, float *post_g, const unsigned *blocks, unsigned long long block_words,
                                   long long rows_pad, int G, int nranks, int own, unsigned cap, uint2 *seen);
hipError_t launch_f32_to_f64(hipStream_t st, const float *in, double *out, long long n);
hipError_t launch_prior_betas(hipStream_t st, const float *betas, float *bsum, const unsigned long long *n_mol,
                              const int *v2snp, const int *snp_ptr, const int *snp_vars, long long V, int G,
                              double default_prior, float *out);
hipError_t launch_rebuild_nz(hipStream_t st, const float *post, long long B, int K, int G, float nz_floor,
                             unsigned long long *nz, uint2 *first);
hipError_t launch_assign(hipStream_t st, const float *post, long long B, int K, int *best, float *best_p);
hipError_t launch_test_log(hipStream_t st, const float *in, float *out, long long n);
hipError_t launch_test_log_hot(hipStream_t st, const float *in, float *out, long long n);
hipError_t launch_test_exp(hipStream_t st, const float *in, float *out, long long n);
hipError_t launch_test_log2_hw(hipStream_t st, const float *in, float *out, long long n);
hipError_t launch_test_softmax(hipStream_t st, const float *in, float *out, long long rows, int cols);

}
```

### demuxalot_amd/csrc/kernels.hip

```cpp
#include <hip/hip_runtime.h>

#include <cstdlib>
#include <cstring>

#include <type_traits>
#include <utility>
#include "kernels.h"
#include "np_math.h"
#include "estep_epilogue.h"

namespace dmx {

template <typename T, int L>
__global__ __launch_bounds__(256) void k_probs_from_betas(const T *__restrict__ prior,
                                                          const T *__restrict__ addition,
                                                          const int *__restrict__ v2snp,
                                                          const int *__restrict__ snp_ptr,
                                                          const int *__restrict__ snp_vars, long long v_begin,
                                                          long long n_rows, long long n_snps, int G,
                                                          const int *__restrict__ prow, float clip_lo, float clip_hi,
                                                          float *__restrict__ prob, unsigned short *__restrict__ prob16)
{
    const int lane = threadIdx.x & 63, li = lane & (L - 1);
    const long long r = ((long long)blockIdx.x * 4 + (threadIdx.x >> 6)) * (64 / L) + lane / L;
// ... 1265 lines not shown
    const long long b = a.order_count != nullptr ? (long long)a.order[blockIdx.x] : (long long)blockIdx.x;
    const int K = a.K, G = a.G;
    const float *__restrict__ lg = a.logits + (size_t)b * K;
    float *post = a.post + (size_t)b * K;
    float mx = -__builtin_inff();
    for (int k0 = tid; k0 < K; k0 += 256 * 8) {
        float v[8];
#pragma unroll
        for (int u = 0; u < 8; u++) v[u] = k0 + 256 * u < K ? lg[k0 + 256 * u] : -__builtin_inff();
#pragma unroll
        for (int u = 0; u < 8; u++) {
            mx = fmaxf(mx, v[u]);
            if (STAGED && k0 + 256 * u < K) sh_row[k0 + 256 * u] = v[u];
        }
    }
#pragma unroll
    for (int off = 1; off < 64; off <<= 1) mx = fmaxf(mx, __shfl_xor(mx, off));
    if (lane == 0) sh_red[wave] = mx;
    __syncthreads();
    mx = fmaxf(fmaxf(sh_red[0], sh_red[1]), fmaxf(sh_red[2], sh_red[3]));
    float *x = STAGED ? sh_row : post;
    for (int k = tid; k < K; k += 256) x[k] = npm::exp_f32((STAGED ? sh_row[k] : lg[k]) - mx);
    __threadfence_block();
    __syncthreads();
    if constexpr (STAGED) {
        const float tot = npm::plan_sum_block<float>(x, a.sum_plan, sh_row + K, tid);
        if (tid == 0) sh_red[4] = tot;
    } else if (wave == 0) {
        const float tot = npm::row_sum_wave(x, K, lane);
        if (lane == 0) sh_red[4] = tot;
    }
    __syncthreads();
    const float tot = sh_red[4];
    const int W = (G + 63) >> 6;
    bool redo = false;
    if (a.guard && guard_active(a)) {
        const bool counting = a.guard == 2;
        const float n = (float)(2 * (a.pair_ptr[b + 1] - a.pair_ptr[b]));
        float dmax = 0.0f;
        bool bad = false;
        for (int k = tid; k < K; k += 256) {
            const float l = lg[k];
            const float d = GUARD_RHO * (fabsf(l) + fabsf(a.pen[k]) + GUARD_POSITIVE_TERM * n) + a.guard_per_call * (n + 8.0f) + GUARD_LOGIT_ROUNDING * fabsf(l);
            bad |= !(d < 0.25f);
            dmax = fmaxf(dmax, d);
        }
#pragma unroll
        for (int off = 1; off < 64; off <<= 1) dmax = fmaxf(dmax, __shfl_xor(dmax, off));
        if (lane == 0) sh_guard[wave] = dmax;
        __syncthreads();
        dmax = fmaxf(fmaxf(sh_guard[0], sh_guard[1]), fmaxf(sh_guard[2], sh_guard[3]));
        const float x2 = 2.0f * dmax;
        const float e2 = x2 * (1.0f + x2) * 1.000001f;
        const float near = mx - (x2 + 2.4e-7f * fabsf(mx)) * 1.000001f;
        int close = 0;
        for (int k = tid; k < K; k += 256) {
            const float p = x[k] / tot;
            bad |= !(fminf(p, 1.0f - p) * e2 <= (K > 1024 ? GUARD_TOL_WIDE : GUARD_TOL));
            close += !(lg[k] < near) ? 1 : 0;
        }
#pragma unroll
        for (int off = 1; off < 64; off <<= 1) close += __shfl_xor(close, off);
        const bool any_bad = __ballot(bad) != 0ull;
        if (lane == 0) {
            sh_guard[4 + wave] = (float)close;
            sh_guard[8 + wave] = any_bad ? 1.0f : 0.0f;
        }
        __syncthreads();
        const float total_close = sh_guard[4] + sh_guard[5] + sh_guard[6] + sh_guard[7];
        const bool flagged = total_close != 1.0f || (sh_guard[8] + sh_guard[9] + sh_guard[10] + sh_guard[11]) != 0.0f;
        if (flagged && tid == 0) guard_note(a, b, counting);
        redo = flagged && !counting;
    }
    for (int k0 = 0; k0 < K; k0 += 256) {
        const int k = k0 + tid;
        float p = 0.0f;
        if (k < K) {
            p = x[k] / tot;
            post[k] = p;
            if (a.post_singlets != nullptr && k < G) a.post_singlets[(size_t)b * G + k] = p;
        }
        if (k0 < G) {
            const unsigned long long bal = __ballot(k < G && !(p <= a.nz_floor));
            const int word = (k0 >> 6) + wave;
            if (lane == 0 && word < W) a.nz[(size_t)b * W + word] = bal;
            if (a.first && word == 0 && lane == (bal ? __builtin_ctzll(bal) : 0)) {
                a.first[b] = nz_code(bal, p);
                if (a.dense_calls && !redo && __popcll(bal) > 4)
                    atomicAdd(a.dense_calls + 1 + (b & (DENSE_SLOTS - 1)), (unsigned long long)(2 * (a.pair_ptr[b + 1] - a.pair_ptr[b])));
            }
        }
    }
}

template <int A, int H, bool SQUARE>
static __device__ __forceinline__ void mstep_terms(const npm::f32x2 (&p)[H][A], const npm::f32x2 (&keep)[H], float power,
                                                   double (&acc)[A])
{
#pragma unroll
    for (int q = 0; q < H; q++) {
#pragma unroll
        for (int s = 0; s < A; s++) {
            npm::f32x2 c = p[q][s] * keep[q];
            if (SQUARE) {
                c = c * c;
            } else {
                c.x = powf(c.x, power);
                c.y = powf(c.y, power);
            }
            acc[s] += (double)c.x;
            acc[s] += (double)c.y;
        }
    }
}

static __device__ __forceinline__ void mstep_store(const MstepArgs &a, long long item, int g, double acc)
{
    if (a.item_variant != nullptr) {
        const long long v = a.item_variant[item];
        if (a.item_ptr[v + 1] - a.item_ptr[v] == 1) {
            const size_t o = (size_t)(a.prow ? (long long)a.prow[v] : v) * a.G + g;
            if (a.out32) a.out32[o] = (float)acc;
            else a.out64[o] = acc;
            return;
        }
    }
    a.partial[(size_t)item * a.G + g] = acc;
}

template <int A, int U, bool SQUARE, bool SMALL>
__global__ __launch_bounds__(256) void k_mstep(MstepArgs a)
{
    static_assert(64 % U == 0, "chunk must be a multiple of the unroll");
    const int lane = threadIdx.x & 63;
    const int G = a.G;
    const int W = (G + 63) >> 6;
    double acc[A];
#pragma unroll
    for (int s = 0; s < A; s++) acc[s] = 0.0;

    const int wave = __builtin_amdgcn_readfirstlane((int)(threadIdx.x >> 6));
    const long long slot = (long long)blockIdx.x * 4 + wave;
    if (slot >= a.n_items) return;
    const long long item = a.order[slot];
    const int n = a.item_len[item];
    const uint2 *__restrict__ calls = a.calls + a.item_start[item];
    const __amdgpu_buffer_rsrc_t rsrc =
        __builtin_amdgcn_make_buffer_rsrc((void *)a.post, 0, SMALL ? (int)a.post_bytes : 0, 0x00020000);
    unsigned voff[A];
#pragma unroll
    for (int s = 0; s < A; s++) voff[s] = (unsigned)(lane + 64 * s) * 4u;

    auto load_records = [&](int c0) {
        const int ci = c0 + lane;
        uint2 d = make_uint2(0u, 0u);
        if (ci < n) d = calls[ci];
        return d;
    };
    auto load_bitmap = [&](int c0, uint2 d, int s) {
        unsigned long long m = 0ull;
        if (c0 + lane < n && s < W) m = a.nz[(size_t)d.x * W + s];
        return m;
    };
    uint2 d_cur = load_records(0);
    uint2 d_nxt = load_records(64);
    unsigned long long m_cur[A], m_nxt[A];
#pragma unroll
    for (int s = 0; s < A; s++) m_cur[s] = load_bitmap(0, d_cur, s);
    for (int c0 = 0; c0 < n; c0 += 64) {
        const uint2 d_nn = load_records(c0 + 128);
#pragma unroll
// ... 153 lines not shown
    st[GS_DIRECT_STEPS] += level == 2u;
    st[GS_COARSE_STEPS] += level == 0u;
    st[GS_STREAK] = streak;
    st[GS_CAPABLE] = capable != 0;
    st[GS_COUNT] = 0u;
    st[GS_ROWS] = B;
    st[GS_K] = K;
    st[GS_VALID] = 1u;
    st[GS_PENDING] = 1u;
    st[GS_T_FAST] = st[GS_T_REDO] = st[GS_T_END] = (unsigned)wall_clock64();
}

hipError_t launch_guard_begin(hipStream_t st, unsigned *state, long long B, int K, int adaptive, int capable, int allow_coarse)
{
    hipLaunchKernelGGL(k_guard_begin, dim3(1), dim3(GUARD_SLOTS), 0, st, state, (unsigned)B, (unsigned)K, adaptive, capable, allow_coarse);
    return hipGetLastError();
}

__global__ __launch_bounds__(256) void k_guard_compact(unsigned *st, const int *__restrict__ sub, unsigned cap, int *__restrict__ list,
                                                       const int *__restrict__ order_direct, unsigned B)
{
    __shared__ unsigned before[4], all[4];
    const unsigned q = blockIdx.x;
    if (st[GS_DIRECT] != 0u) {
        for (unsigned i = q * 256u + threadIdx.x; i < B; i += GUARD_QUEUES * 256u) list[i] = order_direct[i];
        if (q == 0 && threadIdx.x == 0) {
            st[GS_COUNT] = B;
            st[GS_T_REDO] = (unsigned)wall_clock64();
        }
        return;
    }
    const unsigned len = st[GS_QUEUE_LEN + threadIdx.x];
    unsigned lo = threadIdx.x < q ? len : 0u, total = len;
    for (int off = 32; off > 0; off >>= 1) {
        lo += __shfl_down(lo, off);
        total += __shfl_down(total, off);
    }
    if ((threadIdx.x & 63) == 0) {
        before[threadIdx.x >> 6] = lo;
        all[threadIdx.x >> 6] = total;
    }
    __syncthreads();
    const unsigned offset = before[0] + before[1] + before[2] + before[3];
    const unsigned mine = st[GS_QUEUE_LEN + q];
    for (unsigned i = threadIdx.x; i < mine; i += 256) list[offset + i] = sub[(size_t)q * cap + i];
    if (q == 0 && threadIdx.x == 0) {
        st[GS_COUNT] = all[0] + all[1] + all[2] + all[3];
        st[GS_T_REDO] = (unsigned)wall_clock64();
    }
}

hipError_t launch_guard_compact(hipStream_t st, unsigned *state, const int *sub, unsigned sub_cap, int *list, const int *order_direct, long long B)
{
    hipLaunchKernelGGL(k_guard_compact, dim3(GUARD_QUEUES), dim3(256), 0, st, state, sub, sub_cap, list, order_direct, (unsigned)B);
    return hipGetLastError();
}

__global__ void k_guard_stamp(unsigned *st, int which) { st[which] = (unsigned)wall_clock64(); }

hipError_t launch_guard_stamp(hipStream_t st, unsigned *state, int which)
{
    hipLaunchKernelGGL(k_guard_stamp, dim3(1), dim3(1), 0, st, state, which);
    return hipGetLastError();
}

hipError_t launch_sum_dense(hipStream_t st, unsigned long long *counters, unsigned *guard_state)
{
    hipLaunchKernelGGL(k_sum_dense, dim3(1), dim3(256), 0, st, counters, guard_state);
    return hipGetLastError();
}

static __device__ __forceinline__ bool dense_regime(const MstepArgs &a)
{
    return a.dense_calls != nullptr && 4ull * *a.dense_calls > a.total_calls;
}

static __device__ __forceinline__ bool incr_full(const unsigned *state, const MstepArgs &a)
{
    const unsigned long long calls = ((unsigned long long)state[IS_CALLS + 1] << 32) | state[IS_CALLS];
    if (state[IS_FORCE] != 0u) return dense_regime(a);
    return state[IS_VALID] == 0u || 8ull * calls > (a.incr_total ? a.incr_total : a.total_calls) || dense_regime(a);
}

static __device__ __forceinline__ unsigned long long fixed_of(float c, int shift)
{
    constexpr double MAGIC = 6755399441055744.0;
    const double d = __builtin_ldexp((double)c, shift) + MAGIC;
    return (unsigned long long)(__double_as_longlong(d) - __double_as_longlong(MAGIC));
}

static __device__ __forceinline__ void mstep_out_fixed(const MstepArgs &a, long long v, int g, unsigned long long acc, int shift)
{
    const size_t o = (size_t)(a.prow ? (long long)a.prow[v] : v) * a.G + g;
    const double sum = __builtin_ldexp((double)(long long)acc, -shift);
    if (a.out32) a.out32[o] = (float)sum;
    else a.out64[o] = sum;
}

static __device__ __forceinline__ void mstep_store_fixed(const MstepArgs &a, long long item, int g, unsigned long long acc, int shift)
{
    const long long v = a.item_variant[item];
    if (a.item_ptr[v + 1] - a.item_ptr[v] == 1) {
        mstep_out_fixed(a, v, g, acc, shift);
        a.fixed_acc64[(size_t)v * a.G + g] = acc;
        return;
    }
    a.partial[(size_t)item * a.G + g] = __longlong_as_double((long long)acc);
}

template <bool SQUARE>
__global__ __launch_bounds__(256) void k_mstep_dense(MstepArgs a)
{
    if (!dense_regime(a)) return;
    const int lane = threadIdx.x & 63;
    const int wave = __builtin_amdgcn_readfirstlane((int)(threadIdx.x >> 6));
    for (long long slot = (long long)blockIdx.x * 4 + wave; slot < a.n_items; slot += (long long)gridDim.x * 4) {
        const long long item = a.order[slot];
        const int n = a.item_len[item];
        const uint2 *__restrict__ calls = a.calls + a.item_start[item];
        const __amdgpu_buffer_rsrc_t rsrc = __builtin_amdgcn_make_buffer_rsrc((void *)a.post, 0, (int)a.post_bytes, 0x00020000);
        const unsigned row_bytes = (unsigned)a.K * 4u;
        const unsigned voff = (unsigned)(lane < a.G ? lane : 0) * 4u;
        double acc = 0.0;
        auto records = [&](int c0) {
            uint2 d = make_uint2(0u, 0u);
            if (c0 + lane < n) d = calls[c0 + lane];
            return d;
        };
        constexpr int DENSE_ROWS = 16;
        uint2 d_cur = records(0);
        for (int c0 = 0; c0 < n; c0 += 64) {
            const uint2 d_nxt = records(c0 + 64);
            const int cnt = (n - c0) < 64 ? (n - c0) : 64;
            for (int i0 = 0; i0 < cnt; i0 += DENSE_ROWS) {
                float p[DENSE_ROWS];
    #pragma unroll
                for (int u = 0; u < DENSE_ROWS; u++) {
                    const unsigned cb = (unsigned)__builtin_amdgcn_readlane((int)d_cur.x, (i0 + u) & 63);
                    p[u] = __builtin_bit_cast(float, __builtin_amdgcn_raw_buffer_load_b32(rsrc, (int)voff, (int)(cb * row_bytes), 0));
                }
    #pragma unroll
                for (int u = 0; u < DENSE_ROWS; u++) {
                    const float keep = __builtin_bit_cast(float, __builtin_amdgcn_readlane((int)d_cur.y, (i0 + u) & 63));
                    float c = p[u] * keep;
                    c = SQUARE ? c * c : powf(c, a.power);
                    acc += (double)c;
                }
            }
            d_cur = d_nxt;
        }
        if (lane < a.G) mstep_store(a, item, lane, acc);
    }
}

template <bool SQUARE, int R, int D, bool BUF, bool FIXED = false>
__global__ __launch_bounds__(256) void k_mstep_calls(MstepArgs a)
{
    if (dense_regime(a)) return;
    if (FIXED && a.fixed_state != nullptr && !incr_full(a.fixed_state, a)) return;
    constexpr int NZ_S = NZ_CODE;
    typedef unsigned long long u64;
    __shared__ float sh_val[4][R * 64];
    __shared__ u64 sh_colmask[4][64];
    const int lane = threadIdx.x & 63;
    const int wave = __builtin_amdgcn_readfirstlane((int)(threadIdx.x >> 6));
    const long long slot = (long long)blockIdx.x * 4 + wave;
    if (slot >= a.n_items) return;
    const long long item = a.order[slot];
    const int n = a.item_len[item];
    const uint2 *__restrict__ calls = a.calls + a.item_start[item];
    float *val = sh_val[wave];
    u64 *colmask = sh_colmask[wave];
// ... 185 lines not shown
            if (prefetched) {
#pragma unroll
                for (int j = 0; j < DP; j++) {
                    if (todo) {
                        put_dense(__builtin_ctzll(todo), q0[j], cm);
                        todo &= todo - 1ull;
                    }
                }
            }
            while (todo) {
                float q[D];
                load_dense_rows(todo, d0, bm0, q);
#pragma unroll
                for (int j = 0; j < D; j++) {
                    if (todo) {
                        put_dense(__builtin_ctzll(todo), q[j], cm);
                        todo &= todo - 1ull;
                    }
                }
            }
        };

        u64 cm = transpose(mine_all);
        if (!__any(__popcll(cm) + __popcll(dense0) > R)) {
            put_dense_calls(dense0, cm, true);
            colmask[lane] = cm;
            put_sparse(mine_all);
            drain(cm);
        } else {
            int first_lane = 0, width = 32;
            while (first_lane < 64) {
                const u64 range = ((1ull << width) - 1ull) << first_lane;
                const int mine = (range & bit) ? mine_all : 0;
                cm = transpose(mine);
                if (width > R && __any(__popcll(cm) + __popcll(dense0 & range) > R)) {
                    width >>= 1;
                    continue;
                }
                put_dense_calls(dense0 & range, cm, false);
                colmask[lane] = cm;
                put_sparse(mine);
                drain(cm);
                first_lane += width;
            }
        }
        d0 = d1; d1 = d2; d2 = d3;
        fc0 = fc1; fc1 = fc2;
        dense0 = dense1;
        bm0 = bm1;
#pragma unroll
        for (int j = 0; j < DP; j++) q0[j] = q1[j];
#pragma unroll
        for (int t = 0; t < NZ_S; t++) ps0[t] = ps1[t];
    }
    if (lane < G) {
        if constexpr (FIXED) mstep_store_fixed(a, item, lane, acc_fixed, shift);
        else mstep_store(a, item, lane, acc);
    }
}

constexpr int MTILE_THREADS = 1024;
constexpr int MTILE_QUEUE = 96;

template <bool SQUARE>
__global__ __launch_bounds__(MTILE_THREADS) void k_mstep_tiles(MstepArgs a, MTileArgs t)
{
    if (dense_regime(a)) return;
    if (t.incr_state != nullptr && !incr_full(t.incr_state, a)) return;
    extern __shared__ __attribute__((aligned(16))) unsigned long long mt_acc[];
    __shared__ unsigned mt_queue[MTILE_THREADS / 64][2][MTILE_QUEUE];
    const int tile = t.order[blockIdx.x];
    const int v0 = t.first[tile], nv = t.first[tile + 1] - v0;
    const long long beg = t.ptr[tile], end = t.ptr[tile + 1];
    const int G = a.G;
    const long long K = a.K;
    for (int i = threadIdx.x; i < nv * G; i += MTILE_THREADS) mt_acc[i] = 0ull;
    __syncthreads();
    const int lane = threadIdx.x & 63;
    const int wave = __builtin_amdgcn_readfirstlane((int)(threadIdx.x >> 6));
    const int shift = __builtin_amdgcn_readfirstlane(t.shift[tile]);
    unsigned *q_rec = mt_queue[wave][0], *q_keep = mt_queue[wave][1];
    int queued = 0;
    auto power_of = [&](float c) { return SQUARE ? c * c : powf(c, a.power); };
    constexpr double MAGIC = 6755399441055744.0;
    auto add = [&](int index, float c) {
        const double d = __builtin_ldexp((double)c, shift) + MAGIC;
        const unsigned long long q = (unsigned long long)(__double_as_longlong(d) - __double_as_longlong(MAGIC));
        __hip_atomic_fetch_add(&mt_acc[index], q, __ATOMIC_RELAXED, __HIP_MEMORY_SCOPE_WORKGROUP);
    };
    auto flush = [&]() {
        __builtin_amdgcn_fence(__ATOMIC_RELEASE, "wavefront");
        __builtin_amdgcn_wave_barrier();
        __builtin_amdgcn_fence(__ATOMIC_ACQUIRE, "wavefront");
        constexpr int DB = 16;
        for (int q0 = 0; q0 < queued; q0 += DB) {
            float p[DB];
#pragma unroll
            for (int i = 0; i < DB; i++) {
                p[i] = 0.0f;
                if (q0 + i < queued && lane < G) p[i] = a.post[(size_t)(q_rec[q0 + i] & 0xFFFFFFu) * K + lane];
            }
#pragma unroll
            for (int i = 0; i < DB; i++)
                if (q0 + i < queued && lane < G) add((int)(q_rec[q0 + i] >> 24) * G + lane, power_of(p[i] * __uint_as_float(q_keep[q0 + i])));
        }
        __builtin_amdgcn_fence(__ATOMIC_RELEASE, "wavefront");
        __builtin_amdgcn_wave_barrier();
        queued = 0;
    };
    constexpr int UN = 4;
    for (long long c0 = beg + (long long)wave * (64 * UN); c0 < end; c0 += (long long)(MTILE_THREADS / 64) * 64 * UN) {
        uint2 rec[UN], code[UN];
#pragma unroll
        for (int u = 0; u < UN; u++) {
            const long long i = c0 + 64 * u + lane;
            rec[u] = make_uint2(0u, 0u);
            if (i < end) rec[u] = t.stream[i];
        }
#pragma unroll
        for (int u = 0; u < UN; u++) {
            const long long i = c0 + 64 * u + lane;
            code[u] = make_uint2(0u, 0u);
            if (i < end) code[u] = a.first[rec[u].x & 0xFFFFFFu];
        }
        float extra[UN][NZ_CODE - 1];
#pragma unroll
        for (int u = 0; u < UN; u++) {
            const int nnz = (int)(code[u].y & 127u);
            const float *__restrict__ post_row = a.post + (size_t)(rec[u].x & 0xFFFFFFu) * K;
#pragma unroll
            for (int j = 1; j < NZ_CODE; j++) {
                extra[u][j - 1] = 0.0f;
                if (nnz <= NZ_CODE && j < nnz) extra[u][j - 1] = post_row[(code[u].y >> (7 + 6 * j)) & 63u];
            }
        }
#pragma unroll
        for (int u = 0; u < UN; u++) {
            const unsigned row = rec[u].x & 0xFFFFFFu;
            const int base = (int)(rec[u].x >> 24) * G;
            const float keep = __uint_as_float(rec[u].y);
            const int nnz = (int)(code[u].y & 127u);
            if (nnz >= 1 && nnz <= NZ_CODE) {
                add(base + (int)((code[u].y >> 7) & 63u), power_of(__uint_as_float(code[u].x) * keep));
#pragma unroll
                for (int j = 1; j < NZ_CODE; j++)
                    if (j < nnz) add(base + (int)((code[u].y >> (7 + 6 * j)) & 63u), power_of(extra[u][j - 1] * keep));
            }
            const unsigned long long dense = __ballot(nnz > NZ_CODE);
            if (dense) {
                if (queued > MTILE_QUEUE - 64) flush();
                if (nnz > NZ_CODE) {
                    const int at = queued + __popcll(dense & ((1ull << lane) - 1ull));
                    q_rec[at] = rec[u].x;
                    q_keep[at] = rec[u].y;
                }
                queued += __popcll(dense);
            }
        }
    }
    if (queued) flush();
    __syncthreads();
    for (int i = threadIdx.x; i < nv * G; i += MTILE_THREADS) {
        const int r = (int)((unsigned)i / (unsigned)G), g = i - r * G;
        const long long v = v0 + r;
        const size_t o = (size_t)(a.prow ? (long long)a.prow[v] : v) * G + g;
        const double sum = __builtin_ldexp((double)(long long)mt_acc[i], -shift);
        if (a.out32) a.out32[o] = (float)sum;
        else a.out64[o] = sum;
        if (t.acc64) t.acc64[(size_t)v * G + g] = mt_acc[i];
    }
}

constexpr unsigned MINCR_COOLDOWN = 8;
static __device__ __forceinline__ bool mincr_differs(float now, float before, float floor)
{
    return __float_as_uint(now) != __float_as_uint(before) && !(fmaxf(now, before) < floor);
}

__global__ __launch_bounds__(256) void k_mincr_changes(MstepArgs a, MIncrArgs x)
{
    if (x.state[IS_VALID] == 0u || dense_regime(a)) return;
    const int lane = threadIdx.x & 63;
    const long long b = ((long long)blockIdx.x * 4 + (threadIdx.x >> 6)) * 16 + lane;
    bool look = false;
    if (lane < 16 && b < x.B) {
        const uint2 now = a.first[b], before = x.prev_first[b];
        look = !((now.y & 127u) == 1u && now.x == before.x && now.y == before.y);
    }
    for (unsigned long long m = __ballot(look); m != 0ull; m &= m - 1ull) {
        const long long bb = b - lane + __builtin_ctzll(m);
        bool differs = false;
        if (lane < a.G) differs = mincr_differs(a.post[(size_t)bb * a.K + lane], x.prev[(size_t)bb * a.G + lane], x.floor);
        const bool changed = __ballot(differs) != 0ull;
        if (lane == 0) {
            if (changed) {
                x.list[atomicAdd(x.state + IS_N, 1u)] = (int)bb;
                atomicAdd((unsigned long long *)(x.state + IS_CALLS), x.pair_ptr  ? 2ull * (unsigned long long)(x.pair_ptr[bb + 1] - x.pair_ptr[bb])
                                                                    : x.rec_ptr ? (unsigned long long)(x.rec_ptr[bb + 1] - x.rec_ptr[bb])
                                                                                : 2ull);
                if (x.changed_map) x.changed_map[bb] = 1;
            } else {
                x.prev_first[bb] = a.first[bb];
            }
        }
    }
}

template <bool SQUARE>
__global__ __launch_bounds__(256) void k_mincr_delta(MstepArgs a, MIncrArgs x)
{
    if (incr_full(x.state, a)) return;
    const int lane = threadIdx.x & 63;
    const unsigned n = x.state[IS_N];
    const int G = a.G;
    constexpr double MAGIC = 6755399441055744.0;
    auto quant = [&](float c, int shift) {
        const double d = __builtin_ldexp((double)(SQUARE ? c * c : powf(c, a.power)), shift) + MAGIC;
        return (unsigned long long)(__double_as_longlong(d) - __double_as_longlong(MAGIC));
    };
    const int wave = threadIdx.x >> 6;
    for (unsigned i = blockIdx.x; i < n; i += gridDim.x) {
        const long long b = x.list[i];
        float now = 0.0f, before = 0.0f;
        if (lane < G) {
            now = a.post[(size_t)b * a.K + lane];
            before = x.prev[(size_t)b * G + lane];
        }
        const unsigned long long mask = __ballot(lane < G && mincr_differs(now, before, x.floor));
        const bool indexed = x.rec_ptr != nullptr;
        const long long p0 = indexed ? x.rec_ptr[b] : x.pair_ptr[b];
        const int n_calls = indexed ? (int)(x.rec_ptr[b + 1] - p0) : 2 * (int)(x.pair_ptr[b + 1] - p0);
        for (int c0 = 64 * wave; c0 < n_calls; c0 += 256) {
            const int ci = c0 + lane;
            const bool mine = ci < n_calls;
            float keep = 0.0f;
            unsigned row = 0u;
            if (mine && indexed) {
                const uint2 d = x.rec[p0 + ci];
                row = d.x;
                keep = __uint_as_float(d.y);
            } else if (mine) {
                keep = x.pairs[p0 + (ci >> 1)].keep[ci & 1];
                row = x.call_rows != nullptr ? x.call_rows[2 * p0 + ci] : x.pairs[p0 + (ci >> 1)].row_off[ci & 1] / (4u * (unsigned)G);
                if (x.row_variant != nullptr) row = (unsigned)x.row_variant[row];
            }
            const int shift = mine ? (int)x.shift_v[row] : 0;
            for (unsigned long long m = mask; m != 0ull; m &= m - 1ull) {
                const int g = __builtin_ctzll(m);
                const float pn = __shfl(now, g), po = __shfl(before, g);
                const unsigned long long qn = quant(pn * keep, shift), qo = quant(po * keep, shift);
                if (mine && qn != qo) {
                    __hip_atomic_fetch_add(&x.acc64[(size_t)row * G + g], qn - qo, __ATOMIC_RELAXED, __HIP_MEMORY_SCOPE_AGENT);
                    x.touched[row] = 1;
                }
            }
        }
        __syncthreads();
        if (wave == 0) {
            if (lane < G) x.prev[(size_t)b * G + lane] = now;
            if (lane == 0) x.prev_first[b] = a.first[b];
        }
    }
}

template <bool SQUARE>
__global__ __launch_bounds__(256) void k_mincr_delta_masked(MstepArgs a, MIncrArgs x)
{
    if (incr_full(x.state, a)) return;
    const int lane = threadIdx.x & 63;
    const int G = a.G;
    auto quant = [&](float c, int shift) { return fixed_of(SQUARE ? c * c : powf(c, a.power), shift); };
    for (long long slot = (long long)blockIdx.x * 4 + (threadIdx.x >> 6); slot < a.n_items; slot += (long long)gridDim.x * 4) {
        const long long item = a.order[slot];
        const int n = a.item_len[item];
        const uint2 *__restrict__ calls = a.calls + a.item_start[item];
        const long long v = a.item_variant[item];
        const int shift = (int)x.shift_v[v];
        bool touched = false;
        for (int c0 = 0; c0 < n; c0 += 64) {
            uint2 d = make_uint2(0u, 0u);
            bool flagged = false;
            if (c0 + lane < n) {
                d = calls[c0 + lane];
                flagged = x.changed_map[d.x] != 0;
            }
            for (unsigned long long m = __ballot(flagged); m != 0ull; m &= m - 1ull) {
                const int src = __builtin_ctzll(m);
                const unsigned row = (unsigned)__shfl((int)d.x, src);
                const float keep = __uint_as_float((unsigned)__shfl((int)d.y, src));
                if (lane < G) {
                    const float now = a.post[(size_t)row * a.K + lane], before = x.prev[(size_t)row * G + lane];
                    if (mincr_differs(now, before, x.floor)) {
                        const unsigned long long qn = quant(now * keep, shift), qo = quant(before * keep, shift);
                        if (qn != qo) {
                            __hip_atomic_fetch_add(&x.acc64[(size_t)v * G + lane], qn - qo, __ATOMIC_RELAXED, __HIP_MEMORY_SCOPE_AGENT);
                            touched = true;
                        }
                    }
                }
            }
        }
        if (__ballot(touched) != 0ull && lane == 0) x.touched[v] = 1;
// ... 1007 lines not shown
```

### demuxalot_amd/csrc/mstep_plan.h

```cpp
#pragma once

#include <algorithm>

namespace dmx {
namespace mplan {

struct Facts {
    int mstep_tiles;
    int mstep_incremental;
    bool exact_additions;
    int G;
    bool has_calls;
    float power;
    bool attached;
    bool mshard;
    bool sliced;
    bool reduce_f64;
    bool has_call_pairs;
    bool has_item_variant;
    bool has_shift_v;
    bool has_incr_state;
    bool has_slice_rec;
    long long n_mt;
    bool mt_tried;
    long long msteps_done;
    long long msteps_ahead;
    long long msteps_expected;
    bool incr_heavy;
    long long rows_total;
};

inline bool fixed_point_possible(const Facts &f) { return !f.exact_additions && f.G <= 64 && f.has_calls && f.power > 0.0f; }

inline bool own_records(const Facts &f) { return !f.mshard && (!f.attached || f.sliced) && f.has_call_pairs; }

inline bool items_can_start(const Facts &f) { return f.mstep_incremental && fixed_point_possible(f) && own_records(f) && f.has_item_variant; }
inline bool can_go_incremental(const Facts &f) { return f.mstep_tiles == 1 && items_can_start(f); }

constexpr int MSTEP_TILES_PAY = 8;
inline bool probe_step(long long done) { return done == 4 || done == 16 || done == 64; }
inline bool probe_due(const Facts &f)
{
    return can_go_incremental(f) && !f.incr_heavy && f.n_mt == 0 && f.has_incr_state && probe_step(f.msteps_done);
}
inline bool heavy_after_probe(const Facts &f, unsigned full_passes)
{
    return f.msteps_done == 4 ? full_passes >= 3u : 2ull * full_passes >= (unsigned long long)f.msteps_done;
}
inline bool records_wanted(const Facts &f)
{
    const bool long_run = std::max(f.msteps_ahead, f.msteps_expected) >= MSTEP_TILES_PAY || f.msteps_done >= MSTEP_TILES_PAY;
    const bool pays = f.n_mt > 0 || (long_run && (!can_go_incremental(f) || f.incr_heavy));
    return fixed_point_possible(f) && (f.mstep_tiles == 2 || (f.mstep_tiles == 1 && pays));
}
inline bool build_due(const Facts &f) { return records_wanted(f) && !f.mt_tried; }
inline bool tiles_ready(const Facts &f) { return records_wanted(f) && f.n_mt > 0; }

inline bool shifts_wanted(const Facts &f) { return !tiles_ready(f) && f.mstep_tiles != 0 && items_can_start(f); }
enum Incr { INCR_NONE, INCR_OWN_RECORDS, INCR_WORK_ITEMS, INCR_SHARDED };
struct Launch {
    int form;
    Incr incr;
    bool row_variant;
};
inline Launch launch(const Facts &f)
{
    const bool tiles = tiles_ready(f), items = shifts_wanted(f) && f.has_shift_v;
    const bool sharded = tiles && f.mstep_incremental == 1 && f.mshard && f.has_shift_v && f.has_item_variant && f.rows_total > 0;
    const bool own = (tiles || items) && f.mstep_incremental && own_records(f) && f.has_shift_v;
    const Incr incr = sharded ? INCR_SHARDED : !own ? INCR_NONE : items ? INCR_WORK_ITEMS : INCR_OWN_RECORDS;
    return {tiles ? 2 : incr == INCR_WORK_ITEMS ? 3 : 1, incr, own && f.sliced};
}
inline bool sharded_by_row_index(const Facts &f) { return f.has_slice_rec; }
enum Exchange { EXCH_NONE, EXCH_REDUCE_SCATTER, EXCH_ALL_REDUCE };
struct Dest {
    bool exchange_buffer;
    bool f64;
    Exchange then;
    bool slice_only;
};
inline Dest destination(const Facts &f)
{
    if (!f.attached || f.mshard) return {false, false, EXCH_NONE, f.attached};
    if (f.sliced) return {true, f.reduce_f64, EXCH_REDUCE_SCATTER, true};
    return {false, f.reduce_f64, EXCH_ALL_REDUCE, false};
}

struct Range {
    long long v0, v1;
};
inline Range variant_range(const Facts &f, const long long *cut, int rank, long long V)
{
    return f.mshard ? Range{cut[rank], cut[rank + 1]} : Range{0, V};
}

}
}
```

### demuxalot_amd/csrc/repack_device.hip

```cpp
#include <cstring>

#include <cstdlib>
#include <algorithm>
#include <hip/hip_runtime.h>
#include <rocprim/rocprim.hpp>

#include "device_scratch.h"

namespace dmx {
using namespace scratch;
namespace {

__global__ __launch_bounds__(256) void k_validate(const int *__restrict__ variant, const int *__restrict__ cb,
                                                  const float *__restrict__ p_wrong, long long N, long long B, long long V,
                                                  unsigned long long *__restrict__ bad)
{
    const long long i = (long long)blockIdx.x * blockDim.x + threadIdx.x;
    const bool in = i < N;
    const bool bad_b = in && ((unsigned)cb[in ? i : 0] >= (unsigned long long)B);
    const bool bad_v = in && ((unsigned)variant[in ? i : 0] >= (unsigned long long)V);
    const float e = p_wrong[in ? i : 0];
    const bool bad_p = in && !(e >= 0.0f && e <= 1.0f);
    if (__ballot(bad_b || bad_v || bad_p) == 0ull) return;
    if (bad_b || bad_v || bad_p) {
// ... 578 lines not shown
    if (k > n_tiles) return;
    long long lo = 0, hi = n;
    while (lo < hi) {
        const long long mid = (lo + hi) >> 1;
        if ((long long)sorted_keys[mid] < k) lo = mid + 1; else hi = mid;
    }
    ptr[k] = lo;
}
}

void release_mstep_tiles(dmx_ctx *c)
{
    dev_free(c, c->d_mt_stream);
    dev_free(c, c->d_mt_ptr);
    dev_free(c, c->d_mt_first);
    dev_free(c, c->d_mt_order);
    dev_free(c, c->d_mt_shift);
    dev_free(c, c->d_mt_shift_v);
    c->incr_valid = false;
    c->n_mt = 0;
    c->mt_tv = 0;
    c->mt_tried = false;
    c->mt_shift_tried = false;
}

namespace {
struct TileCut {
    std::vector<int> tile_first;
    std::vector<long long> tile_ptr;
    std::vector<unsigned> tile_of, vin_of;
    std::vector<int> tile_shift;
    int tv = 0;
    unsigned row_bits = 0;
    long long n_mt = 0;
};

bool cut_mstep_tiles(dmx_ctx *c, long long v_lo, long long v_hi, TileCut &t)
{
    const int G = c->G;
    const long long rows = c->mshard ? c->rows_total : c->B, m = c->n_csc;
    if (G < 1 || G > 64 || rows >= (1LL << 24) || m == 0 || m >= (1LL << 32) || v_hi <= v_lo) return false;
    const long long V = c->V;
    if ((long long)c->h_col_ptr.size() != V + 1 || c->h_col_ptr[(size_t)V] != m) return false;
    const std::vector<long long> &first_call = c->h_col_ptr;
    if (first_call[(size_t)v_lo] != 0 || first_call[(size_t)v_hi] != m) return false;
    if (!c->n_simd) {
        int cus = 0;
        if (hipDeviceGetAttribute(&cus, hipDeviceAttributeMultiprocessorCount, c->device) != hipSuccess) return false;
        c->n_simd = 4 * cus;
    }
    t.tv = std::max(1, std::min<int>(dmx::MTILE_MAX_VARIANTS, dmx::MTILE_LDS_BYTES / (G * 8)));
    t.row_bits = bits_of(rows ? (unsigned long long)rows - 1 : 0);
    t.tile_of.assign((size_t)V, 0u);
    t.vin_of.assign((size_t)V, 0u);
    long long cap = std::max<long long>(4096, m / std::max(1, c->n_simd));
    for (int attempt = 0;; attempt++) {
        t.tile_first.clear();
        t.tile_ptr.clear();
        long long v = v_lo;
        while (v < v_hi) {
            t.tile_first.push_back((int)v);
            t.tile_ptr.push_back(first_call[(size_t)v]);
            long long w = v + 1;
            while (w < v_hi && w - v < t.tv && first_call[(size_t)w + 1] - first_call[(size_t)v] <= cap) w++;
            for (long long x = v; x < w; x++) {
                t.tile_of[(size_t)x] = (unsigned)(t.tile_first.size() - 1);
                t.vin_of[(size_t)x] = (unsigned)(x - v);
            }
            v = w;
        }
        const unsigned tile_bits = bits_of(t.tile_first.empty() ? 0 : (unsigned long long)t.tile_first.size() - 1);
        if (tile_bits + t.row_bits <= 32) break;
        if (cap >= m || attempt > 40) return false;
        cap *= 2;
    }
    t.n_mt = (long long)t.tile_first.size();
    t.tile_first.push_back((int)v_hi);
    t.tile_ptr.push_back(m);
    t.tile_shift.resize((size_t)t.n_mt);
    for (long long i = 0; i < t.n_mt; i++) {
        long long longest = 1;
        for (long long v = t.tile_first[(size_t)i]; v < t.tile_first[(size_t)i + 1]; v++)
            longest = std::max(longest, first_call[(size_t)v + 1] - first_call[(size_t)v]);
        t.tile_shift[(size_t)i] = std::min(50, 62 - (int)bits_of((unsigned long long)longest));
    }
    return true;
}

int upload_variant_shifts(dmx_ctx *c, const TileCut &t)
{
    const long long V = c->V;
    std::vector<unsigned char> shift_v((size_t)V);
    for (long long v = 0; v < V; v++) shift_v[(size_t)v] = (unsigned char)t.tile_shift[(size_t)t.tile_of[(size_t)v]];
    if (!c->d_mt_shift_v.p) DMX_TRY(dev_alloc(c, c->d_mt_shift_v, (size_t)V));
    HIP_TRY(hipMemcpyAsync(c->d_mt_shift_v.p, shift_v.data(), (size_t)V, hipMemcpyHostToDevice, c->stream));
    HIP_TRY(hipStreamSynchronize(c->stream));
    return 0;
}
}

namespace {
__global__ __launch_bounds__(256) void k_slice_rows(const uint2 *__restrict__ csc, const long long *__restrict__ item_start, const int *__restrict__ item_len,
                                                    const int *__restrict__ item_variant, long long n_items, unsigned *__restrict__ keys,
                                                    unsigned long long *__restrict__ vals)
{
    const long long item = (long long)blockIdx.x * 4 + (threadIdx.x >> 6);
    if (item >= n_items) return;
    const long long s0 = item_start[item];
    const unsigned long long v = (unsigned long long)(unsigned)item_variant[item];
    for (int i = threadIdx.x & 63; i < item_len[item]; i += 64) {
        const uint2 d = csc[s0 + i];
        keys[s0 + i] = d.x;
        vals[s0 + i] = v | ((unsigned long long)d.y << 32);
    }
}
}

int build_slice_row_index(dmx_ctx *c)
{
    if (c->d_slice_rec.p != nullptr || c->slice_index_tried) return 0;
    c->slice_index_tried = true;
    const char *env = std::getenv("DEMUXALOT_AMD_SLICE_INDEX");
    if (env && atoi(env) == 0) return 0;
    const long long m = c->n_csc, rows = c->rows_total;
    if (!c->mshard || m == 0 || rows == 0 || m >= (1LL << 32) || c->d_item_variant.p == nullptr) return 0;
    hipStream_t st = c->stream;
    Scratch sc(c);
    unsigned *keys = nullptr, *keys_out = nullptr;
    unsigned long long *vals = nullptr;
    DMX_TRY(sc.get(&keys, (size_t)m));
    DMX_TRY(sc.get(&keys_out, (size_t)m));
    DMX_TRY(sc.get(&vals, (size_t)m));
    hipLaunchKernelGGL(k_slice_rows, dim3((unsigned)((c->n_items + 3) / 4)), dim3(256), 0, st, c->d_csc.p, c->d_item_start.p, c->d_item_len.p,
                       c->d_item_variant.p, c->n_items, keys, vals);
    DMX_TRY(dev_alloc(c, c->d_slice_rec, (size_t)m));
    DMX_TRY(sort_pairs(sc, keys, keys_out, vals, (unsigned long long *)c->d_slice_rec.p, (size_t)m, bits_of((unsigned long long)(rows - 1)), st));
    DMX_TRY(dev_alloc(c, c->d_slice_ptr, (size_t)rows + 1));
    hipLaunchKernelGGL(k_tile_ptr, dim3(grid_for(rows + 1)), dim3(256), 0, st, keys_out, m, rows, c->d_slice_ptr.p);
    HIP_TRY(hipGetLastError());
    HIP_TRY(hipStreamSynchronize(st));
    return 0;
}

int plan_mstep_shifts(dmx_ctx *c)
{
    if (c->d_mt_shift_v.p != nullptr || c->mt_shift_tried) return 0;
    c->mt_shift_tried = true;
    if (c->mshard) return 0;
    TileCut t;
    if (!cut_mstep_tiles(c, 0, c->V, t)) return 0;
    return upload_variant_shifts(c, t);
}

int build_mstep_tiles(dmx_ctx *c, long long v_lo, long long v_hi)
{
    release_mstep_tiles(c);
    c->mt_tried = true;
    TileCut cut;
    if (!cut_mstep_tiles(c, v_lo, v_hi, cut)) return 0;
    const int G = c->G;
    const long long m = c->n_csc;
    hipStream_t st = c->stream;
    const long long V = c->V;
    const int tv = cut.tv;
    const unsigned row_bits = cut.row_bits;
    std::vector<int> &tile_first = cut.tile_first;
    std::vector<long long> &tile_ptr = cut.tile_ptr;
// ... 442 lines not shown
```

### demuxalot_amd/device.py

```python
import ctypes
import os
import threading

import numpy as np

from . import _lib
from ._lib import DMX_F32, DMX_F64, as_c, check, ptr


DEFAULT_ESTEP_MODE = 'guarded'


class DeviceContext:
    def __init__(self, device=0):
        self._lib = _lib.load()
        handle = ctypes.c_void_p()
        check(self._lib.dmx_create(int(device), ctypes.byref(handle)))
        self._h = handle
        self.device = int(device)
        self.B = self.V = self.G = self.N = 0
        self.K = 0
        self._resident_key = None
        self._keep_molecule_calls = False
        self._snp_shape = (0, 0)
        self.apply_environment()

    def apply_environment(self):
        mode = os.environ.get('DEMUXALOT_AMD_ESTEP', '') or DEFAULT_ESTEP_MODE
        assert mode in ('exact', 'fast', 'guarded'), f'DEMUXALOT_AMD_ESTEP={mode!r}: exact, fast or guarded'
        self.set_estep_mode(mode)
        exact_additions = os.environ.get('DEMUXALOT_AMD_EXACT_ADDITIONS', '')
        self.set_exact_additions(mode == 'exact' if exact_additions == '' else exact_additions != '0')
        self.set_estep_schedule(os.environ.get('DEMUXALOT_AMD_ESTEP_SCHEDULE', 'auto'))
        self.set_estep_dictionary(os.environ.get('DEMUXALOT_AMD_ESTEP_DICT', 'auto'))
        self.set_estep_packing(os.environ.get('DEMUXALOT_AMD_ESTEP_PACKED', 'auto'))
        self.set_coarse_pass(os.environ.get('DEMUXALOT_AMD_COARSE_PASS', '1') != '0')
        self.set_mstep_incremental(os.environ.get('DEMUXALOT_AMD_MSTEP_INCREMENTAL', '1') != '0')
        self.set_lean_memory(os.environ.get('DEMUXALOT_AMD_LEAN', '0') not in ('', '0'))
        self.set_phase_timers(False)
        self.set_logits_needed(True)

    def __enter__(self):
        return self

    def __exit__(self, *_exc):
        self.close()

    def close(self):
        if getattr(self, '_h', None):
            self._lib.dmx_destroy(self._h)
            self._h = None

    def __del__(self):
        try:
            self.close()
        except Exception:
            pass

    def set_problem(self, n_barcodes, n_variants, n_genotypes, variant_id, compressed_cb, p_base_wrong, v2snp):
        self._resident_key = None
        variant_id = as_c(variant_id, np.int32)
        compressed_cb = as_c(compressed_cb, np.int32)
        p_base_wrong = as_c(p_base_wrong, np.float32)
        v2snp = as_c(v2snp, np.int32)
        assert len(variant_id) == len(compressed_cb) == len(p_base_wrong)
        assert len(v2snp) == n_variants
        check(self._lib.dmx_set_problem(self._h, n_barcodes, n_variants, n_genotypes, len(variant_id),
                                        ptr(variant_id), ptr(compressed_cb), ptr(p_base_wrong), ptr(v2snp)))
        self.B, self.V, self.G, self.N = int(n_barcodes), int(n_variants), int(n_genotypes), len(variant_id)

    @staticmethod
    def _variant_arrays(var_chrom, var_pos, var_base, v2snp):
        var_chrom, var_pos, var_base = as_c(var_chrom, np.int32), as_c(var_pos, np.int32), as_c(var_base, np.uint8)
        v2snp = as_c(v2snp, np.int32)
        assert len(v2snp) == len(var_pos)
        return var_chrom, var_pos, var_base, v2snp

    def _pack(self, entry, n_barcodes, n_genotypes, variants, *calls):
        n_variants = len(variants[1])
        mol_per_variant = np.zeros(n_variants, dtype=np.int64)
        n_matched, n_unique = ctypes.c_int64(0), ctypes.c_int64(0)
        check(entry(self._h, n_barcodes, n_variants, n_genotypes, *(ptr(a) for a in variants), *calls,
                    ctypes.byref(n_matched), ctypes.byref(n_unique), ptr(mol_per_variant)))
        self.B, self.V, self.G, self.N = int(n_barcodes), int(n_variants), int(n_genotypes), n_unique.value
        return n_matched.value, n_unique.value, mol_per_variant

    def pack_and_set_problem(self, n_barcodes, n_genotypes, var_chrom, var_pos, var_base, v2snp,
                             call_chrom, call_pos, call_base, call_cb, call_p):
        self._resident_key = None
        variants = self._variant_arrays(var_chrom, var_pos, var_base, v2snp)
        call_chrom, call_pos = as_c(call_chrom, np.int32), as_c(call_pos, np.int32)
        call_base, call_cb, call_p = as_c(call_base, np.uint8), as_c(call_cb, np.int32), as_c(call_p, np.float32)
        return self._pack(self._lib.dmx_pack_and_set_problem, n_barcodes, n_genotypes, variants, len(call_pos),
                          ptr(call_chrom), ptr(call_pos), ptr(call_base), ptr(call_cb), ptr(call_p))

    def _container_list(self, containers):
        from .snp_counter import MOLECULE_DTYPE, SNP_CALL_DTYPE

        class Container(ctypes.Structure):
            _fields_ = [('snp_calls', ctypes.c_void_p), ('n_snp_calls', ctypes.c_int64),
                        ('molecules', ctypes.c_void_p), ('n_molecules', ctypes.c_int64), ('chrom', ctypes.c_int32)]

        keep_alive, parts = [], (Container * max(1, len(containers)))()
        for k, (chrom, snp_calls, molecules) in enumerate(containers):
            assert snp_calls.dtype == SNP_CALL_DTYPE and molecules.dtype == MOLECULE_DTYPE
            snp_calls, molecules = np.ascontiguousarray(snp_calls), np.ascontiguousarray(molecules)
            keep_alive += [snp_calls, molecules]
            parts[k] = Container(snp_calls.ctypes.data, len(snp_calls), molecules.ctypes.data, len(molecules), int(chrom))
        return parts, keep_alive

    def pack_containers_and_set_problem(self, n_barcodes, n_genotypes, var_chrom, var_pos, var_base, v2snp, containers):
        self._resident_key = None
        variants = self._variant_arrays(var_chrom, var_pos, var_base, v2snp)
        parts, _keep_alive = self._container_list(containers)
        return self._pack(self._lib.dmx_pack_containers_and_set_problem, n_barcodes, n_genotypes, variants,
                          ctypes.cast(parts, ctypes.c_void_p), len(containers))

    def stage_containers(self, containers):
        self._resident_key = None
        parts, _keep_alive = self._container_list(containers)
        check(self._lib.dmx_stage_containers(self._h, ctypes.cast(parts, ctypes.c_void_p), len(containers)))
# ... 543 lines not shown

    def set_guard_adaptive(self, adaptive):
        check(self._lib.dmx_set_guard_adaptive(self._h, int(bool(adaptive))))

    def set_coarse_pass(self, coarse):
        check(self._lib.dmx_set_coarse_pass(self._h, 2 if coarse == 'always' else int(bool(coarse))))

    def set_lean_memory(self, lean):
        check(self._lib.dmx_set_lean_memory(self._h, int(bool(lean))))

    def set_mstep_incremental(self, incremental):
        check(self._lib.dmx_set_mstep_incremental(self._h, 2 if incremental == 'bootstrap' else int(bool(incremental))))

    def mstep_incremental(self):
        full, delta, last = ctypes.c_int64(), ctypes.c_int64(), ctypes.c_int64()
        check(self._lib.dmx_get_mstep_incremental(self._h, ctypes.byref(full), ctypes.byref(delta), ctypes.byref(last)))
        return full.value, delta.value, last.value

    def guard_levels(self):
        level = ctypes.c_int32()
        steps, fine, coarse = ctypes.c_int64(), ctypes.c_int64(), ctypes.c_int64()
        c_ms, f_ms, e_ms = ctypes.c_double(), ctypes.c_double(), ctypes.c_double()
        check(self._lib.dmx_get_guard_levels(self._h, ctypes.byref(level), ctypes.byref(steps), ctypes.byref(fine), ctypes.byref(coarse),
                                             ctypes.byref(c_ms), ctypes.byref(f_ms), ctypes.byref(e_ms)))
        return {'level': level.value, 'coarse_steps': steps.value, 'flagged_fine': fine.value, 'flagged_coarse': coarse.value,
                'coarse_pass_ms': c_ms.value, 'fine_pass_ms': f_ms.value, 'exact_pass_ms': e_ms.value}

    def set_logits_needed(self, needed):
        check(self._lib.dmx_set_logits_needed(self._h, int(bool(needed))))

    def guard_probes(self):
        probes, streak = ctypes.c_int64(), ctypes.c_int64()
        check(self._lib.dmx_get_guard_probes(self._h, ctypes.byref(probes), ctypes.byref(streak)))
        return probes.value, streak.value

    def debug_set_pass_ms(self, coarse=-1.0, fine=-1.0, exact=-1.0):
        check(self._lib.dmx_debug_set_pass_ms(self._h, float(coarse), float(fine), float(exact)))

    def guard_direct(self):
        return self.guard_state()[:3]

    def guard_state(self):
        last, steps, would = ctypes.c_int32(0), ctypes.c_int64(0), ctypes.c_int64(0)
        fast_ms, exact_ms = ctypes.c_double(0), ctypes.c_double(0)
        check(self._lib.dmx_get_guard_direct(self._h, ctypes.byref(last), ctypes.byref(steps), ctypes.byref(would),
                                             ctypes.byref(fast_ms), ctypes.byref(exact_ms)))
        return bool(last.value), steps.value, would.value, fast_ms.value, exact_ms.value

    def set_estep_dictionary(self, mode):
        check(self._lib.dmx_set_estep_dictionary(self._h, {'never': 0, 'auto': 1, 'always': 2}[mode]))

    def estep_form(self):
        form, distinct = ctypes.c_int32(0), ctypes.c_int32(0)
        check(self._lib.dmx_get_estep_form(self._h, ctypes.byref(form), ctypes.byref(distinct)))
        return {0: None, 1: 'direct', 2: 'dict', 3: 'dict_block', 4: 'packed'}[form.value], distinct.value

    def set_estep_packing(self, mode):
        check(self._lib.dmx_set_estep_packing(self._h, {'never': 0, 'auto': 1, 'always': 2, 'split': 3}[mode]))

    def set_estep_schedule(self, schedule):
        check(self._lib.dmx_set_estep_schedule(self._h, {'direct': 0, 'auto': 1, 'tiled': 2}[schedule]))

    def set_mstep_wide_addresses(self, wide):
        check(self._lib.dmx_set_mstep_wide_addresses(self._h, int(bool(wide))))

    def set_mstep_tiles(self, mode):
        if isinstance(mode, str):
            mode = {'never': 0, 'auto': 1, 'always': 2}[mode]
        check(self._lib.dmx_set_mstep_tiles(self._h, int(mode) if not isinstance(mode, bool) else (2 if mode else 0)))

    def set_msteps_expected(self, n):
        check(self._lib.dmx_set_msteps_expected(self._h, int(n)))

    def mstep_tiles_info(self):
        built, ms = ctypes.c_int32(0), ctypes.c_double(0)
        check(self._lib.dmx_get_mstep_tiles_info(self._h, ctypes.byref(built), ctypes.byref(ms)))
        return bool(built.value), ms.value

    def mstep_form(self):
        form = ctypes.c_int32(0)
        check(self._lib.dmx_get_mstep_form(self._h, ctypes.byref(form)))
        return {0: None, 1: 'items', 2: 'tiles', 3: 'items_fixed'}[form.value]

    def redo_count(self):
        n = ctypes.c_int64(0)
        check(self._lib.dmx_get_redo_count(self._h, ctypes.byref(n)))
        return n.value

    def set_exact_additions(self, exact):
        check(self._lib.dmx_set_exact_additions(self._h, int(bool(exact))))

    def set_phase_timers(self, on):
        check(self._lib.dmx_set_phase_timers(self._h, int(bool(on))))

    def timings(self):
        ms = (ctypes.c_double * _lib.T_COUNT)()
        n = (ctypes.c_int64 * _lib.T_COUNT)()
        check(self._lib.dmx_get_timings(self._h, ms, n))
        return {name: dict(ms=ms[i], launches=int(n[i])) for i, name in enumerate(_lib.TIMER_NAMES)}

    def reset_timings(self):
        check(self._lib.dmx_reset_timings(self._h))

    def trim_cache(self):
        n = ctypes.c_int64(0)
        check(self._lib.dmx_trim_cache(self._h, ctypes.byref(n)))
        return n.value

    def release_problem(self):
        self._resident_key = None
        check(self._lib.dmx_release_problem(self._h))
        self.B = self.V = self.G = self.N = self.K = 0

    def device_bytes(self):
        n = ctypes.c_int64(0)
        check(self._lib.dmx_device_bytes(self._h, ctypes.byref(n)))
        return n.value

    def test_log(self, x):
        x = as_c(x, np.float32)
        out = np.empty_like(x)
        check(self._lib.dmx_test_logf(self._h, ptr(x), ptr(out), x.size))
        return out

    def test_log_hot(self, x):
        x = as_c(x, np.float32)
        out = np.empty_like(x)
        check(self._lib.dmx_test_logf_hot(self._h, ptr(x), ptr(out), x.size))
        return out

    def test_log2_hw(self, x):
        x = as_c(x, np.float32)
        out = np.empty_like(x)
        check(self._lib.dmx_test_log2_hw(self._h, ptr(x), ptr(out), x.size))
        return out

    def test_exp(self, x):
        x = as_c(x, np.float32)
        out = np.empty_like(x)
        check(self._lib.dmx_test_expf(self._h, ptr(x), ptr(out), x.size))
        return out

    def test_softmax(self, x):
        x = as_c(x, np.float32)
        out = np.empty_like(x)
        check(self._lib.dmx_test_softmax(self._h, ptr(x), ptr(out), x.shape[0], x.shape[1]))
        return out


_contexts = {}
_contexts_lock = threading.RLock()


def default_device():
    if os.environ.get('DEMUXALOT_AMD_DEVICE', '') != '':
        return int(os.environ['DEMUXALOT_AMD_DEVICE'])
    if os.environ.get('LOCAL_RANK', '') != '':
        n = _lib.device_count()
        return int(os.environ['LOCAL_RANK']) % n if n > 0 else 0
    return 0


def get_context(device=None) -> DeviceContext:
    device = default_device() if device is None else int(device)
    with _contexts_lock:
        if device not in _contexts:
# ... 59 lines not shown
```

### include/demux_hip_debug.h

```cpp
#ifndef DEMUX_HIP_DEBUG_H
#define DEMUX_HIP_DEBUG_H

#include "demux_hip.h"

#ifdef __cplusplus
extern "C" {
#endif

int dmx_get_redo_count(dmx_ctx *ctx, int64_t *count);

int dmx_set_mstep_tiles(dmx_ctx *ctx, int enable);
int dmx_get_mstep_tiles_info(dmx_ctx *ctx, int32_t *built, double *build_ms);
int dmx_get_mstep_form(dmx_ctx *ctx, int32_t *form);

int dmx_set_guard_adaptive(dmx_ctx *ctx, int adaptive);
int dmx_set_coarse_pass(dmx_ctx *ctx, int coarse);

int dmx_set_mstep_incremental(dmx_ctx *ctx, int incremental);
int dmx_get_mstep_incremental(dmx_ctx *ctx, int64_t *full_passes, int64_t *delta_passes, int64_t *barcodes_changed_last);
int dmx_get_guard_levels(dmx_ctx *ctx, int32_t *level_last, int64_t *coarse_steps, int64_t *flagged_fine_last, int64_t *flagged_coarse_last,
                         double *coarse_pass_ms, double *fine_pass_ms, double *exact_pass_ms);
int dmx_get_guard_probes(dmx_ctx *ctx, int64_t *probes, int64_t *streak);
int dmx_debug_set_pass_ms(dmx_ctx *ctx, double coarse_pass_ms, double fine_pass_ms, double exact_pass_ms);
int dmx_get_guard_direct(dmx_ctx *ctx, int32_t *last_ran_direct, int64_t *direct_steps, int64_t *would_queue_last, double *fast_pass_ms,
                         double *exact_pass_ms);

int dmx_set_estep_schedule(dmx_ctx *ctx, int tiled);

#define DMX_FORM_NONE 0
#define DMX_FORM_DIRECT 1
#define DMX_FORM_DICT 2
#define DMX_FORM_DICT_BLOCK 3
#define DMX_FORM_PACKED 4
int dmx_set_estep_dictionary(dmx_ctx *ctx, int mode);
int dmx_get_estep_form(dmx_ctx *ctx, int32_t *form, int32_t *distinct_values);

int dmx_set_estep_packing(dmx_ctx *ctx, int mode);

int dmx_set_mstep_wide_addresses(dmx_ctx *ctx, int wide);

int dmx_comm_init_emulated(dmx_ctx *ctx, int rank, int nranks, double link_gbytes_per_s, double latency_us, int reduce_dtype);

int dmx_get_exchange_compact(dmx_ctx *ctx, int64_t *taken, int64_t *overflows, int64_t *capacity_rows);
int dmx_get_exchange_compact_table(dmx_ctx *ctx, int64_t *taken, int64_t *overflows, int64_t *capacity_rows);

int dmx_test_logf(dmx_ctx *ctx, const float *in, float *out, int64_t n);
int dmx_test_logf_hot(dmx_ctx *ctx, const float *in, float *out, int64_t n);
int dmx_test_expf(dmx_ctx *ctx, const float *in, float *out, int64_t n);
int dmx_test_log2_hw(dmx_ctx *ctx, const float *in, float *out, int64_t n);
int dmx_test_softmax(dmx_ctx *ctx, const float *in, float *out, int64_t rows, int64_t cols);

int dmx_get_guard_stats(dmx_ctx *ctx, int64_t *redone_last, int64_t *redone_total, int64_t *rows_total);

#define DMX_EXCHANGE_NONE 0
#define DMX_EXCHANGE_VARIANT 1
#define DMX_EXCHANGE_REDUCE_SCATTER 2
#define DMX_EXCHANGE_ALLREDUCE 3
int dmx_get_exchange_mode(dmx_ctx *ctx, int32_t *mode);

int dmx_runtime_info(char *out, int64_t capacity);

int dmx_count_reads_begin(dmx_ctx *ctx, const int32_t *positions, int64_t n_positions, const double *qual_table41);
int dmx_count_reads_push(dmx_ctx *ctx, const dmx_decoded_reads *chunk, int final, int64_t *n_molecules, int64_t *n_calls);
int dmx_count_reads_end(dmx_ctx *ctx);

int dmx_get_count_reads_timings(dmx_ctx *ctx, double *stage_ms);
int dmx_get_count_reads_carry(dmx_ctx *ctx, int64_t *n_reads);
int dmx_get_count_reads_peak_bytes(dmx_ctx *ctx, int64_t *bytes);

#define DMX_COVERAGE_ATOMIC 0
#define DMX_COVERAGE_TILED 1
int dmx_set_coverage_form(dmx_ctx *ctx, int form);
int dmx_get_coverage_timings(dmx_ctx *ctx, double *stage_ms);

int dmx_reads_upload(dmx_ctx *ctx, const dmx_decoded_reads *reads, int64_t *handle);
int dmx_reads_release(dmx_ctx *ctx, int64_t handle);
int dmx_reads_info(dmx_ctx *ctx, int64_t handle, int64_t *info);
int dmx_count_reads_resident(dmx_ctx *ctx, int64_t handle, const int32_t *positions, int64_t n_positions, const double *qual_table41,
                             int64_t *n_molecules, int64_t *n_calls);
int dmx_coverage_count_resident(dmx_ctx *ctx, int64_t handle, int32_t start, int32_t stop, int32_t quality_threshold,
                                int32_t *coverage_out);
int dmx_count_reads_push_resident(dmx_ctx *ctx, int64_t handle, int64_t first_read, int64_t last_read, int final, int64_t *n_molecules,
                                  int64_t *n_calls);
int dmx_get_reads_upload_bytes(dmx_ctx *ctx, int64_t *bytes);

int dmx_calls_upload(dmx_ctx *ctx, const dmx_call_container *host, int64_t *handle);
int dmx_calls_open(dmx_ctx *ctx, int64_t *handle);
int dmx_calls_append_counted(dmx_ctx *ctx, int64_t handle);
int dmx_calls_seal(dmx_ctx *ctx, int64_t handle);
int dmx_calls_concatenate(dmx_ctx *ctx, const int64_t *handles, int32_t n_handles, int64_t *handle);
int dmx_calls_view(dmx_ctx *ctx, int64_t handle, dmx_call_container *view);
int dmx_calls_info(dmx_ctx *ctx, int64_t handle, int64_t *info);
int dmx_calls_fetch(dmx_ctx *ctx, int64_t handle, void *molecules_out, void *snp_calls_out);
int dmx_calls_release(dmx_ctx *ctx, int64_t handle);
int dmx_calls_barcode_counts(dmx_ctx *ctx, int64_t handle, int64_t n_barcodes, int64_t *calls_per_barcode, int64_t *molecules_per_barcode);
int dmx_stage_device_containers(dmx_ctx *ctx, const dmx_call_container *views, int32_t n_views);
// ... 32 lines not shown
```

Baseline: 185.4 million.

## Raise E-step live-posterior floor to fixed-point grid when M-step sums on grid

When the M-step accumulates in fixed point (tiles, shifts), posteriors below the smallest representable quantum contribute zero. The E-step therefore marks them non-live using a higher floor, so sparse per-barcode live sets shrink and the M-step touches fewer entries. The dense-regime statistic still uses the old floor, and the nz codes are rebuilt if the plan falls back to a non-grid form. The tile kernel also skips atomics for zero quantized values. This adds planning logic and a possible extra rebuild pass, and it risks mismatches if the planner's prediction differs between the E-step and the M-step.

```diff
diff --git a/demuxalot_amd/_lib.py b/demuxalot_amd/_lib.py
--- a/demuxalot_amd/_lib.py
+++ b/demuxalot_amd/_lib.py
@@ -106,6 +106,9 @@
     'dmx_set_mstep_tiles': (c_int, [_P, c_int]),
     'dmx_get_mstep_form': (c_int, [_P, POINTER(c_int32)]),
     'dmx_get_mstep_tiles_info': (c_int, [_P, POINTER(c_int32), POINTER(c_double)]),
+    'dmx_set_live_floor_on_grid': (c_int, [_P, c_int]),
+    'dmx_get_live_floor': (c_int, [_P, POINTER(c_float), POINTER(c_int64)]),
+    'dmx_debug_get_live_counts': (c_int, [_P, _P]),
     'dmx_test_logf': (c_int, [_P, _P, _P, c_int64]),
     'dmx_test_logf_hot': (c_int, [_P, _P, _P, c_int64]),
     'dmx_test_expf': (c_int, [_P, _P, _P, c_int64]),
diff --git a/demuxalot_amd/csrc/dmx_api.cpp b/demuxalot_amd/csrc/dmx_api.cpp
--- a/demuxalot_amd/csrc/dmx_api.cpp
+++ b/demuxalot_amd/csrc/dmx_api.cpp
@@ -451,6 +451,34 @@
 {
     if (!c || !form) return fail(DMX_ERR_INVALID, "null argument");
     *form = c->mstep_form;
+    return 0;
+}
+
+int dmx_set_live_floor_on_grid(dmx_ctx *c, int on_grid)
+{
+    if (!c) return fail(DMX_ERR_INVALID, "null context");
+    c->live_floor_grid = on_grid != 0;
+    return 0;
+}
+
+int dmx_get_live_floor(dmx_ctx *c, float *floor, int64_t *rebuilds)
+{
+    if (!c) return fail(DMX_ERR_INVALID, "null context");
+    if (floor) *floor = c->nz_floor;
+    if (rebuilds) *rebuilds = (int64_t)c->nz_rebuilds;
+    return 0;
+}
+
+int dmx_debug_get_live_counts(dmx_ctx *c, int32_t *counts)
+{
+    DMX_TRY(bind(c));
+    DMX_TRY(need(c, c->have_problem && c->have_post, "an E-step before dmx_debug_get_live_counts"));
+    if (c->G > 64 || c->mshard) return fail(DMX_ERR_UNSUPPORTED, "dmx_debug_get_live_counts: barcode codes exist for G <= 64 on a context that holds its own");
+    if (!counts && c->B > 0) return fail(DMX_ERR_INVALID, "null argument");
+    std::vector<uint2> codes((size_t)c->B);
+    if (c->B) HIP_TRY(hipMemcpyAsync(codes.data(), c->d_first.p, sizeof(uint2) * (size_t)c->B, hipMemcpyDeviceToHost, c->stream));
+    HIP_TRY(hipStreamSynchronize(c->stream));
+    for (long long b = 0; b < c->B; b++) counts[b] = (int32_t)(codes[(size_t)b].y & 127u);
     return 0;
 }
 
diff --git a/demuxalot_amd/csrc/dmx_ctx.h b/demuxalot_amd/csrc/dmx_ctx.h
--- a/demuxalot_amd/csrc/dmx_ctx.h
+++ b/demuxalot_amd/csrc/dmx_ctx.h
@@ -204,6 +204,8 @@
     DevBuf<double> d_seg_sums;
     long long n_segs = 0, n_split = 0;
     float nz_floor = 0.0f;
+    int live_floor_grid = 1;
+    long long nz_rebuilds = 0;
     DevBuf<uint2> d_first;
     DevBuf<unsigned long long> d_dense_calls;
     bool dense_stat_valid = false;
diff --git a/demuxalot_amd/csrc/dmx_runtime.cpp b/demuxalot_amd/csrc/dmx_runtime.cpp
--- a/demuxalot_amd/csrc/dmx_runtime.cpp
+++ b/demuxalot_amd/csrc/dmx_runtime.cpp
@@ -783,6 +783,7 @@
     if (c->d_guard_count.p) HIP_TRY(hipMemsetAsync(c->d_guard_count.p + dmx::GS_COARSE_STEPS, 0, 2 * sizeof(unsigned), c->stream));
     if (c->d_incr_state.p) HIP_TRY(hipMemsetAsync(c->d_incr_state.p + 2 * dmx::IS_WORDS, 0, sizeof(unsigned) * 3, c->stream));
     c->guard_rows_total = 0;
+    c->nz_rebuilds = 0;
     for (int s = 0; s < DMX_T_COUNT; s++) {
         timer_flush(c, s);
         c->timers[s].ms = 0.0;
diff --git a/demuxalot_amd/csrc/dmx_steps.cpp b/demuxalot_amd/csrc/dmx_steps.cpp
--- a/demuxalot_amd/csrc/dmx_steps.cpp
+++ b/demuxalot_amd/csrc/dmx_steps.cpp
@@ -319,6 +319,35 @@
     return 0;
 }
 
+static mplan::Facts mstep_facts(const dmx_ctx *c, float power)
+{
+    mplan::Facts f{};
+    f.mstep_tiles = c->mstep_tiles;
+    f.mstep_incremental = c->mstep_incremental;
+    f.exact_additions = c->exact_additions;
+    f.G = c->G;
+    f.has_calls = c->n_csc > 0;
+    f.power = power;
+    f.attached = c->attached();
+    f.mshard = c->mshard;
+    f.sliced = c->sliced;
+    f.reduce_f64 = c->reduce_dtype == DMX_F64;
+    f.has_call_pairs = c->d_call_pairs.p != nullptr;
+    f.has_item_variant = c->d_item_variant.p != nullptr;
+    f.has_shift_v = c->d_mt_shift_v.p != nullptr;
+    f.has_incr_state = c->d_incr_state.p != nullptr;
+    f.has_slice_rec = c->d_slice_rec.p != nullptr;
+    f.n_mt = c->n_mt;
+    f.mt_tried = c->mt_tried;
+    f.msteps_done = c->msteps_done;
+    f.msteps_ahead = c->msteps_ahead;
+    f.msteps_expected = c->msteps_expected;
+    f.incr_heavy = c->incr_heavy;
+    f.rows_total = c->rows_total;
+    f.shift_tried = c->mt_shift_tried;
+    return f;
+}
+
 static void fill_estep_args(dmx_ctx *c, dmx::EstepArgs &a, int with_doublets, bool with_prior, int prior_dtype, float power)
 {
     a.pair_ptr = c->d_pair_ptr.p;
@@ -348,7 +377,8 @@
     a.first = c->G <= 64 ? (c->mshard ? c->d_first_g.p + row_base : c->d_first.p) : nullptr;
     a.post_singlets = c->mshard ? c->d_post_g.p + row_base * c->G : nullptr;
     a.dense_calls = c->G <= 64 ? c->d_dense_calls.p : nullptr;
-    a.nz_floor = power == 2.0f ? dmx::NZ_FLOOR_SQUARE : 0.0f;
+    a.dense_floor = dmx::live_floor_float64(power);
+    a.nz_floor = c->live_floor_grid && mplan::live_floor_on_grid(mstep_facts(c, power)) ? dmx::live_floor_fixed(power) : a.dense_floor;
     a.B = c->B;
     a.prob_bytes = (unsigned)((unsigned long long)c->prob_rows * c->G * 4ull);
     a.G = c->G;
@@ -583,39 +613,20 @@
     a.power = power;
     a.dense_calls = c->dense_stat_valid && a.post_bytes < (1ull << 32) ? c->d_dense_calls.p : nullptr;
     a.total_calls = 2ull * (unsigned long long)c->n_pairs;
-    if (!a.square && c->nz_floor != 0.0f) {
-        HIP_TRY(dmx::launch_rebuild_nz(c->stream, c->d_post.p, c->B, c->K, c->G, 0.0f, (mshard ? c->d_nz_g.p : c->d_nz.p) + row_base * Wn,
+    auto rebuild_codes = [&](float floor) -> int {
+        HIP_TRY(dmx::launch_rebuild_nz(c->stream, c->d_post.p, c->B, c->K, c->G, floor, (mshard ? c->d_nz_g.p : c->d_nz.p) + row_base * Wn,
                                        c->G <= 64 ? (mshard ? c->d_first_g.p : c->d_first.p) + row_base : nullptr));
-        c->nz_floor = 0.0f;
+        c->nz_floor = floor;
         c->post_gathered = false;
-    }
+        c->nz_rebuilds++;
+        return 0;
+    };
+    if (!a.square && c->nz_floor != 0.0f) DMX_TRY(rebuild_codes(0.0f));
     DMX_TRY(gather_posteriors(c));
     c->add_is_zero = false;
     TimerSpan ev{nullptr, nullptr};
     SpanGuard ev_guard{c, &ev};
-    mplan::Facts f{};
-    f.mstep_tiles = c->mstep_tiles;
-    f.mstep_incremental = c->mstep_incremental;
-    f.exact_additions = c->exact_additions;
-    f.G = c->G;
-    f.has_calls = c->n_csc > 0;
-    f.power = power;
-    f.attached = c->attached();
-    f.mshard = c->mshard;
-    f.sliced = c->sliced;
-    f.reduce_f64 = c->reduce_dtype == DMX_F64;
-    f.has_call_pairs = c->d_call_pairs.p != nullptr;
-    f.has_item_variant = c->d_item_variant.p != nullptr;
-    f.has_shift_v = c->d_mt_shift_v.p != nullptr;
-    f.has_incr_state = c->d_incr_state.p != nullptr;
-    f.has_slice_rec = c->d_slice_rec.p != nullptr;
-    f.n_mt = c->n_mt;
-    f.mt_tried = c->mt_tried;
-    f.msteps_done = c->msteps_done;
-    f.msteps_ahead = c->msteps_ahead;
-    f.msteps_expected = c->msteps_expected;
-    f.incr_heavy = c->incr_heavy;
-    f.rows_total = c->rows_total;
+    mplan::Facts f = mstep_facts(c, power);
     if (mplan::probe_due(f)) {
         unsigned full_passes = 0;
         HIP_TRY(hipMemcpyAsync(&full_passes, c->d_incr_state.p + 2 * dmx::IS_WORDS + 3, sizeof(unsigned), hipMemcpyDeviceToHost, c->stream));
@@ -636,6 +647,7 @@
     f.has_shift_v = c->d_mt_shift_v.p != nullptr;
     const mplan::Launch plan = mplan::launch(f);
     const mplan::Dest dest = mplan::destination(f);
+    if (!mplan::grid_floor_admitted(plan) && c->nz_floor > dmx::live_floor_float64(power)) DMX_TRY(rebuild_codes(dmx::live_floor_float64(power)));
     const bool incremental = plan.incr != mplan::INCR_NONE, sharded = plan.incr == mplan::INCR_SHARDED;
     const long long incr_rows = sharded ? c->rows_total : c->B;
     if (incremental) DMX_TRY(ensure_incremental_state(c, sharded, incr_rows, power));
@@ -938,13 +950,11 @@
     for (int it = 0; it < n_iterations; it++) {
         const bool kept = it + 1 == n_iterations && keep_last;
         DMX_TRY(run_pstep(c, lo, hi, true, !kept && it > 0 && ep::coarse_capable(estep_facts(c, with_doublets, false, kept), lo)));
-        DMX_TRY(run_estep(c, with_doublets, it == 0 && prior_logits != nullptr, prior_dtype, power, kept));
-        if (it + 1 < n_iterations) {
-            c->msteps_ahead = n_iterations - 1 - it;
-            const int rc_m = run_mstep(c, power);
-            c->msteps_ahead = 0;
-            if (rc_m) return rc_m;
-        }
+        c->msteps_ahead = n_iterations - 1 - it;
+        const int rc_e = run_estep(c, with_doublets, it == 0 && prior_logits != nullptr, prior_dtype, power, kept);
+        const int rc_m = rc_e == 0 && it + 1 < n_iterations ? run_mstep(c, power) : rc_e;
+        c->msteps_ahead = 0;
+        if (rc_m) return rc_m;
     }
     const size_t bk = (size_t)c->B * c->K;
     DMX_TRY(copy_out(c, logits_out, c->d_logits.p, bk));
@@ -996,9 +1006,9 @@
     for (int it = 0; it < n_iterations; it++) {
         const bool kept = it + 1 == n_iterations && c->logits_needed;
         DMX_TRY(run_pstep(c, lo, hi, true, !kept && ep::coarse_capable(estep_facts(c, with_doublets, false, kept), lo)));
-        DMX_TRY(run_estep(c, with_doublets, false, DMX_F32, power, kept));
         c->msteps_ahead = n_iterations - it;
-        const int rc_m = run_mstep(c, power);
+        const int rc_e = run_estep(c, with_doublets, false, DMX_F32, power, kept);
+        const int rc_m = rc_e == 0 ? run_mstep(c, power) : rc_e;
         c->msteps_ahead = 0;
         if (rc_m) return rc_m;
     }
diff --git a/demuxalot_amd/csrc/estep_epilogue.h b/demuxalot_amd/csrc/estep_epilogue.h
--- a/demuxalot_amd/csrc/estep_epilogue.h
+++ b/demuxalot_amd/csrc/estep_epilogue.h
@@ -260,6 +260,7 @@
     const float tot = reg_row_sum<L, A>(x, K, lane, gbase);
     const int W = (a.G + 63) >> 6;
     unsigned long long mine = 0ull;
+    unsigned long long mine_stat = 0ull;
     float post[A];
 #pragma unroll
     for (int s = 0; s < A; s++) {
@@ -270,12 +271,15 @@
             a.post[o] = post[s];
             if (a.post_singlets != nullptr && kk[s] < a.G) a.post_singlets[(size_t)b * a.G + kk[s]] = post[s];
         }
-        const unsigned long long bal = __ballot(live && valid[s] && (li + L * s) < a.G && !(post[s] <= a.nz_floor));
+        const bool singlet = live && valid[s] && (li + L * s) < a.G;
+        const unsigned long long bal = __ballot(singlet && !(post[s] <= a.nz_floor));
+        const unsigned long long bal_stat = __ballot(singlet && !(post[s] <= a.dense_floor));
         if (L == 64) {
             if (lane == 0 && s < W) a.nz[(size_t)b * W + s] = bal;
-            if (s == 0) mine = bal;
+            if (s == 0) mine = bal, mine_stat = bal_stat;
         } else if (L * s < 64) {
             mine |= ((bal >> gbase) & group_mask<L>()) << ((L * s) & 63);
+            mine_stat |= ((bal_stat >> gbase) & group_mask<L>()) << ((L * s) & 63);
         }
     }
     if (L < 64 && live && li == 0) a.nz[(size_t)b] = mine;
@@ -310,7 +314,7 @@
 #pragma unroll
         for (int s = 1; s < A; s++) p0 = (g0 >> log2_lanes<L>()) == s ? post[s] : p0;
         if (live && li == (g0 & (L - 1))) a.first[b] = nz_code(mine, p0);
-        if (a.dense_calls && live && !redo && li == 0 && __popcll(mine) > 4)
+        if (a.dense_calls && live && !redo && li == 0 && __popcll(mine_stat) > 4)
             atomicAdd(a.dense_calls + 1 + (b & (DENSE_SLOTS - 1)), (unsigned long long)row_calls);
     }
 }
diff --git a/demuxalot_amd/csrc/fixed_point.h b/demuxalot_amd/csrc/fixed_point.h
--- /dev/null
+++ b/demuxalot_amd/csrc/fixed_point.h
@@ -0,0 +1,20 @@
+#pragma once
+
+#if defined(__HIPCC__)
+#define DMX_FIXED_HD __host__ __device__
+#else
+#define DMX_FIXED_HD
+#endif
+
+namespace dmx {
+
+constexpr int FIXED_SHIFT_MAX = 50;
+
+DMX_FIXED_HD inline unsigned long long fixed_of(float c, int shift)
+{
+    constexpr double MAGIC = 6755399441055744.0;
+    const double d = __builtin_ldexp((double)c, shift) + MAGIC;
+    return (unsigned long long)(__builtin_bit_cast(long long, d) - __builtin_bit_cast(long long, MAGIC));
+}
+
+}
diff --git a/demuxalot_amd/csrc/kernels.h b/demuxalot_amd/csrc/kernels.h
--- a/demuxalot_amd/csrc/kernels.h
+++ b/demuxalot_amd/csrc/kernels.h
@@ -1,9 +1,12 @@
 #pragma once
 #include <hip/hip_runtime.h>
+
+#include <cmath>
 
 #include "demux_hip.h"
 #include "demux_hip_debug.h"
 #include "estep_plan.h"
+#include "fixed_point.h"
 
 namespace dmx {
 
@@ -91,6 +94,7 @@
     long long n_long;
     const float *dict;
     const unsigned char *codes;
+    float dense_floor;
 };
 
 enum { GS_COUNT = 0,
@@ -184,6 +188,7 @@
 };
 
 constexpr float NZ_FLOOR_SQUARE = 8.271806125530277e-25f;
+inline float live_floor_float64(float power) { return power == 2.0f ? NZ_FLOOR_SQUARE : 0.0f; }
 
 constexpr int MIN_ITEM_CALLS = 1024, MAX_ITEM_CALLS = 16384;
 inline int item_calls_for(long long n_calls)
@@ -253,6 +258,8 @@
        IS_FORCE = 7,
        IS_WORDS = 8 };
 inline float mincr_floor(float power) { return power * 126.0f > 52.0f ? exp2f(-52.0f / power) : 0.0f; }
+constexpr float KEEP_MAX = 1.0f;
+inline float live_floor_fixed(float power) { return power == 2.0f ? nextafterf(mincr_floor(power) / KEEP_MAX, 0.0f) : live_floor_float64(power); }
 hipError_t launch_mstep_incremental(hipStream_t st, const MstepArgs &a, const MTileArgs *t, const MIncrArgs &x);
 constexpr int MTILE_LDS_BYTES = 64 * 1024;
 constexpr int MTILE_MAX_VARIANTS = 128;
diff --git a/demuxalot_amd/csrc/kernels.hip b/demuxalot_amd/csrc/kernels.hip
--- a/demuxalot_amd/csrc/kernels.hip
+++ b/demuxalot_amd/csrc/kernels.hip
@@ -1371,11 +1371,12 @@
         }
         if (k0 < G) {
             const unsigned long long bal = __ballot(k < G && !(p <= a.nz_floor));
+            const unsigned long long bal_stat = __ballot(k < G && !(p <= a.dense_floor));
             const int word = (k0 >> 6) + wave;
             if (lane == 0 && word < W) a.nz[(size_t)b * W + word] = bal;
             if (a.first && word == 0 && lane == (bal ? __builtin_ctzll(bal) : 0)) {
                 a.first[b] = nz_code(bal, p);
-                if (a.dense_calls && !redo && __popcll(bal) > 4)
+                if (a.dense_calls && !redo && __popcll(bal_stat) > 4)
                     atomicAdd(a.dense_calls + 1 + (b & (DENSE_SLOTS - 1)), (unsigned long long)(2 * (a.pair_ptr[b + 1] - a.pair_ptr[b])));
             }
         }
@@ -1695,12 +1696,6 @@
     return state[IS_VALID] == 0u || 8ull * calls > (a.incr_total ? a.incr_total : a.total_calls) || dense_regime(a);
 }
 
-static __device__ __forceinline__ unsigned long long fixed_of(float c, int shift)
-{
-    constexpr double MAGIC = 6755399441055744.0;
-    const double d = __builtin_ldexp((double)c, shift) + MAGIC;
-    return (unsigned long long)(__double_as_longlong(d) - __double_as_longlong(MAGIC));
-}
 
 static __device__ __forceinline__ void mstep_out_fixed(const MstepArgs &a, long long v, int g, unsigned long long acc, int shift)
 {
@@ -2052,11 +2047,12 @@
     unsigned *q_rec = mt_queue[wave][0], *q_keep = mt_queue[wave][1];
     int queued = 0;
     auto power_of = [&](float c) { return SQUARE ? c * c : powf(c, a.power); };
-    constexpr double MAGIC = 6755399441055744.0;
     auto add = [&](int index, float c) {
-        const double d = __builtin_ldexp((double)c, shift) + MAGIC;
-        const unsigned long long q = (unsigned long long)(__double_as_longlong(d) - __double_as_longlong(MAGIC));
-        __hip_atomic_fetch_add(&mt_acc[index], q, __ATOMIC_RELAXED, __HIP_MEMORY_SCOPE_WORKGROUP);
+        __hip_atomic_fetch_add(&mt_acc[index], fixed_of(c, shift), __ATOMIC_RELAXED, __HIP_MEMORY_SCOPE_WORKGROUP);
+    };
+    auto add_nonzero = [&](int index, float c) {
+        const unsigned long long q = fixed_of(c, shift);
+        if (q != 0ull) __hip_atomic_fetch_add(&mt_acc[index], q, __ATOMIC_RELAXED, __HIP_MEMORY_SCOPE_WORKGROUP);
     };
     auto flush = [&]() {
         __builtin_amdgcn_fence(__ATOMIC_RELEASE, "wavefront");
@@ -2072,7 +2068,7 @@
             }
 #pragma unroll
             for (int i = 0; i < DB; i++)
-                if (q0 + i < queued && lane < G) add((int)(q_rec[q0 + i] >> 24) * G + lane, power_of(p[i] * __uint_as_float(q_keep[q0 + i])));
+                if (q0 + i < queued && lane < G) add_nonzero((int)(q_rec[q0 + i] >> 24) * G + lane, power_of(p[i] * __uint_as_float(q_keep[q0 + i])));
         }
         __builtin_amdgcn_fence(__ATOMIC_RELEASE, "wavefront");
         __builtin_amdgcn_wave_barrier();
@@ -2183,11 +2179,7 @@
     const int lane = threadIdx.x & 63;
     const unsigned n = x.state[IS_N];
     const int G = a.G;
-    constexpr double MAGIC = 6755399441055744.0;
-    auto quant = [&](float c, int shift) {
-        const double d = __builtin_ldexp((double)(SQUARE ? c * c : powf(c, a.power)), shift) + MAGIC;
-        return (unsigned long long)(__double_as_longlong(d) - __double_as_longlong(MAGIC));
-    };
+    auto quant = [&](float c, int shift) { return fixed_of(SQUARE ? c * c : powf(c, a.power), shift); };
     const int wave = threadIdx.x >> 6;
     for (unsigned i = blockIdx.x; i < n; i += gridDim.x) {
         const long long b = x.list[i];
diff --git a/demuxalot_amd/csrc/mstep_plan.h b/demuxalot_amd/csrc/mstep_plan.h
--- a/demuxalot_amd/csrc/mstep_plan.h
+++ b/demuxalot_amd/csrc/mstep_plan.h
@@ -28,6 +28,7 @@
     long long msteps_expected;
     bool incr_heavy;
     long long rows_total;
+    bool shift_tried;
 };
 
 inline bool fixed_point_possible(const Facts &f) { return !f.exact_additions && f.G <= 64 && f.has_calls && f.power > 0.0f; }
@@ -71,6 +72,13 @@
     const Incr incr = sharded ? INCR_SHARDED : !own ? INCR_NONE : items ? INCR_WORK_ITEMS : INCR_OWN_RECORDS;
     return {tiles ? 2 : incr == INCR_WORK_ITEMS ? 3 : 1, incr, own && f.sliced};
 }
+inline bool sums_on_grid(const Facts &f)
+{
+    return tiles_ready(f) || build_due(f) || (shifts_wanted(f) && (f.has_shift_v || !f.shift_tried));
+}
+inline bool live_floor_on_grid(const Facts &f) { return !f.attached && sums_on_grid(f); }
+inline bool grid_floor_admitted(const Launch &l) { return l.form != 1; }
+
 inline bool sharded_by_row_index(const Facts &f) { return f.has_slice_rec; }
 enum Exchange { EXCH_NONE, EXCH_REDUCE_SCATTER, EXCH_ALL_REDUCE };
 struct Dest {
diff --git a/demuxalot_amd/csrc/repack_device.hip b/demuxalot_amd/csrc/repack_device.hip
--- a/demuxalot_amd/csrc/repack_device.hip
+++ b/demuxalot_amd/csrc/repack_device.hip
@@ -684,7 +684,7 @@
         long long longest = 1;
         for (long long v = t.tile_first[(size_t)i]; v < t.tile_first[(size_t)i + 1]; v++)
             longest = std::max(longest, first_call[(size_t)v + 1] - first_call[(size_t)v]);
-        t.tile_shift[(size_t)i] = std::min(50, 62 - (int)bits_of((unsigned long long)longest));
+        t.tile_shift[(size_t)i] = std::min(FIXED_SHIFT_MAX, 62 - (int)bits_of((unsigned long long)longest));
     }
     return true;
 }
diff --git a/demuxalot_amd/device.py b/demuxalot_amd/device.py
--- a/demuxalot_amd/device.py
+++ b/demuxalot_amd/device.py
@@ -37,6 +37,7 @@
         self.set_coarse_pass(os.environ.get('DEMUXALOT_AMD_COARSE_PASS', '1') != '0')
         self.set_mstep_incremental(os.environ.get('DEMUXALOT_AMD_MSTEP_INCREMENTAL', '1') != '0')
         self.set_lean_memory(os.environ.get('DEMUXALOT_AMD_LEAN', '0') not in ('', '0'))
+        self.set_live_floor_on_grid(os.environ.get('DEMUXALOT_AMD_LIVE_FLOOR_GRID', '1') != '0')
         self.set_phase_timers(False)
         self.set_logits_needed(True)
 
@@ -746,6 +747,19 @@
         check(self._lib.dmx_get_mstep_form(self._h, ctypes.byref(form)))
         return {0: None, 1: 'items', 2: 'tiles', 3: 'items_fixed'}[form.value]
 
+    def set_live_floor_on_grid(self, on_grid):
+        check(self._lib.dmx_set_live_floor_on_grid(self._h, int(bool(on_grid))))
+
+    def live_floor(self):
+        floor, rebuilds = ctypes.c_float(0), ctypes.c_int64(0)
+        check(self._lib.dmx_get_live_floor(self._h, ctypes.byref(floor), ctypes.byref(rebuilds)))
+        return floor.value, rebuilds.value
+
+    def debug_live_counts(self):
+        out = np.empty(self.B, dtype=np.int32)
+        check(self._lib.dmx_debug_get_live_counts(self._h, out.ctypes.data_as(ctypes.c_void_p)))
+        return out
+
     def redo_count(self):
         n = ctypes.c_int64(0)
         check(self._lib.dmx_get_redo_count(self._h, ctypes.byref(n)))
diff --git a/include/demux_hip_debug.h b/include/demux_hip_debug.h
--- a/include/demux_hip_debug.h
+++ b/include/demux_hip_debug.h
@@ -12,6 +12,9 @@
 int dmx_set_mstep_tiles(dmx_ctx *ctx, int enable);
 int dmx_get_mstep_tiles_info(dmx_ctx *ctx, int32_t *built, double *build_ms);
 int dmx_get_mstep_form(dmx_ctx *ctx, int32_t *form);
+int dmx_set_live_floor_on_grid(dmx_ctx *ctx, int on_grid);
+int dmx_get_live_floor(dmx_ctx *ctx, float *floor, int64_t *rebuilds);
+int dmx_debug_get_live_counts(dmx_ctx *ctx, int32_t *counts);
 
 int dmx_set_guard_adaptive(dmx_ctx *ctx, int adaptive);
 int dmx_set_coarse_pass(dmx_ctx *ctx, int coarse);
```

After: 202.7 million, median of 6. 1.09x the previous value.
